# 3DTopia/3DTopia-XL

Measured on AMD Instinct MI355X. Metric: DiT denoise-steps/sec (N_prim=2048) + samples/sec @25-step DDIM, higher is better.
Workload: dtype f16

## Files before the change

3dtopia-xl_amd/_lib.py:

```python
from __future__ import annotations

import ctypes as C
import os
from typing import Optional

_HERE = os.path.dirname(os.path.abspath(__file__))
LIB_PATH = os.environ.get("PRIMX_LIB") or os.path.join(_HERE, "csrc", "libprimx_hip.so")

F32, F16, BF16 = 0, 1, 2
ACT_NONE, ACT_GELU_TANH, ACT_GELU_ERF = 0, 1, 2
HEADS_ROWS, HEADS_VT, HEADS_KROWS = 0, 1, 2
ABI_VERSION = 30

_p, _i, _l, _f, _d = C.c_void_p, C.c_int, C.c_int64, C.c_float, C.c_double



class DitBlockFold(C.Structure):
    _fields_ = [(n, _p) for n in ("w_q", "b_q", "w_cproj", "b_cproj", "w_qkv", "w_proj", "b_proj", "w_fc1", "w_fc2", "b_fc2",
                                  "Kc", "Vc", "Kb", "Vb", "uv_q", "uv_qkv", "uv_fc1",
                                  "carry_q", "carry_cproj", "carry_fc1", "carry_fc2")] + \
               [(n, _l) for n in ("carry_q_bytes", "carry_cproj_bytes", "carry_fc1_bytes", "carry_fc2_bytes")]


class F32outProblem(C.Structure):
    _fields_ = [("A", _p), ("W", _p), ("bias", _p), ("out", _p), ("N", _i), ("first_wg", _i)]


class DitForwardFold(C.Structure):
    _fields_ = [(n, _i) for n in ("dtype", "Be", "N", "D", "H", "dh", "hidden", "depth", "L", "nq_pad", "nkv_pad_c", "nkv_pad_b",
                                  "b_from", "step", "n_steps")] + \
               [("ln_eps", _f), ("scale", _f)] + \
               [(n, _p) for n in ("h", "xn", "att", "hid", "Qc", "Qs", "Ks", "Vs", "mod", "center0", "center1", "part")] + \
               [(n, _p) for n in ("kv_A", "kv_W", "kv_bias")] + [(n, _i) for n in ("kv_rows", "kv_rows_per_batch", "kv_K")]


SIGNATURES = {
    "primx_dit_blocks_fold": [C.POINTER(DitForwardFold), C.POINTER(DitBlockFold), _p],
    "primx_abi_version": [],
    "primx_last_error": [],
    "primx_last_gemm_kernel": [],
    "primx_padded_head_dim": [_i],
    "primx_layernorm_modulate": [_p, _p, _p, _l, _p, _i, _i, _i, _i, _f, _p, _l, _p, _l, _p],
    "primx_timestep_embedding": [_p, _p, _p, _i, _i, _p],
    "primx_compute_raydirs": [_p, _p, _p, _p, _p, _f, _p, _p, _p, _i, _i, _i, _p],
    "primx_raymarch": [_p, _p, _p, _f, _p, _p, _p, _p, _p, _i, _i, _i, _i, _i, _i, _i, _f, _f, _p],
    "primx_primsdf_query": [_p, _p, _p, _p, _p, _i, _i, _i, _i, _i, _p],
    "primx_vit_tokens": [_p, _p, _p, _p, _p, _i, _i, _i, _i, _p],
    "primx_point_features": [_p, _l, _p, _p, _l, _i, _i, _p],
    "primx_prefetch": [_p, _l, _p],
    "primx_silu_cast": [_p, _p, _i, _l, _p],
    "primx_cast16": [_p, _p, _i, _l, _p],
    "primx_linear_f32": [_p, _p, _p, _p, _p, _i, _i, _i, _i, _p],
    "primx_linear": [_p, _p, _p, _p, _i, _i, _i, _i, _i, _f, _p, _l, _p],
    "primx_linear_gate_residual": [_p, _p, _p, _p, _l, _p, _i, _i, _i, _i, _i, _p, _l, _p],
    "primx_linear_gate_residual_ln": [_p, _p, _p, _p, _l, _p, _i, _i, _i, _i, _p, _p, _l, _p, _f, _p, _l, _i, _p, _l, _p],
    "primx_ln_sync_timeouts": [],
    "primx_linear_f32out": [_p, _p, _p, _p, _i, _i, _i, _i, _i, _p],
    "primx_row_stats": [_p, _i, _i, _f, _p, _p],
    "primx_linear_gate_residual_fold": [_p, _p, _p, _p, _l, _p, _i, _i, _i, _i, _p, _l, _p, _p, _p, _i, _p, _l, _p],
    "primx_linear_heads_fold": [_p, _p, _i, _i, _i, _i, _i, _i, _i, C.POINTER(_i), C.POINTER(_p), _i, _f, _p, _p, _p, _p, _p, _f,
                                _i, _p, _l, _p],
    "primx_linear_heads_fold_pair": [_p, _p, _i, _i, _i, _i, _i, _i, _i, C.POINTER(_i), C.POINTER(_p), _i, _f, _p, _p, _p, _p, _p, _f,
                                     _p, _p, _p, _i, _i, _i, _i, _i, _i, _i, C.POINTER(_i), C.POINTER(_p), _i, _f, _i, _p],
    "primx_linear_f32out_group": [_p, _i, _i, _i, _i, _i, _i, _p],
    "primx_linear_fold": [_p, _p, _p, _i, _i, _i, _i, _p, _p, _p, _p, _p, _f, _i, _p, _l, _p],
    "primx_linear_heads": [_p, _p, _p, _i, _i, _i, _i, _i, _i, _i, C.POINTER(_i), C.POINTER(_p), _i, _i, _i, _f, _i, _p, _l, _p],
    "primx_attention": [_p, _p, _p, _p, _i, _i, _i, _i, _i, _i, _i, _f, _i, _p],
    "primx_attention_bcast": [_p, _p, _p, _p, _i, _i, _i, _i, _i, _i, _i, _f, _p, _p, _i, _i, _i, _p],
    "primx_pack_heads": [_p, _l, _l, _l, _p, _i, _i, _i, _i, _i, _i, _i, _p],
    "primx_cfg_combine": [_p, _p, _i, _l, _f, _p],
    "primx_diffusion_step": [_p, _p, _i, _l, _i, _i, _p, _i, _i, _i, _i, _i, _p, _p, _p, _p],
    "primx_groupnorm_silu": [_p, _p, _p, _p, _i, _i, _i, _i, _f, _i, _i, _p],
    "primx_conv3d_k3": [_p, _p, _p, _p, _f, _p, _i, _i, _i, _i, _i, _i, _p],
    "primx_conv3d_s4_pack": [_p, _p, _i, _i, _p],
    "primx_conv3d_s4_packed": [_p, _p, _p, _p, _f, _p, _i, _i, _i, _p],
    "primx_conv3d_s8_pack": [_p, _p, _p, _i, _p],
    "primx_conv3d_s8_fused": [_p, _p, _p, _p, _p, _p, _p, _f, _p, _p, _p, _i, _i, _p],
    "primx_conv3d_s8_packed": [_p, _p, _p, _p, _f, _p, _i, _i, _p],
    "primx_convtranspose_s4_pack": [_p, _p, _i, _p],
    "primx_convtranspose_s4_packed": [_p, _p, _p, _p, _p, _i, _i, _p],
    "primx_conv3d_s8c32_pack": [_p, _p, _i, _i, _i, _p],
    "primx_conv3d_s8c32_packed": [_p, _p, _p, _p, _p, _f, _p, _f, _p, _i, _i, _i, _p],
    "primx_linear_residual": [_p, _p, _p, _p, _f, _p, _i, _i, _i, _i, _p],
    "primx_conv_in": [_p, _f, _f, _p, _p, _p, _i, _i, _i, _i, _p],
    "primx_convtranspose_k2s2": [_p, _p, _p, _p, _i, _i, _i, _i, _i, _p],
    "primx_vae_output": [_p, _p, _i, _i, _i, _i, _f, _i, _p],
    "primx_latent_denorm": [_p, _p, _p, _f, _p, _p, _l, _i, _i, _p],
    "primx_gemm_f32": [_p, _p, _p, _p, _i, _i, _i, _i, _f, _p, _l, _i, _p],
    "primx_attention_f32": [_p, _p, _p, _p, _i, _i, _i, _i, _i, C.POINTER(_l), C.POINTER(_l), C.POINTER(_l), _f, _p],
    "primx_layernorm_modulate_f32": [_p, _p, _p, _l, _p, _i, _i, _i, _f, _p],
    "primx_silu_f32": [_p, _p, _l, _p],
    "primx_mcubes_workspace": [_i, _i, _i, C.POINTER(_l)],
    "primx_mcubes_count": [_p, _i, _i, _i, _f, _p, _l, _p, _p],
    "primx_mcubes_emit": [_p, _i, _i, _i, _f, _p, _l, _l, _l, _p, _p, _p, _p],
    "primx_noise_filter": [_p, _i, _p, _p],
    "primx_texbake_labels": [_p, _p, _p, _i, _i, _p, _p],
    "primx_texbake_components_workspace": [_i, _i, C.POINTER(_l)],
    "primx_texbake_components": [_p, _i, _i, _p, _l, _p, C.POINTER(_l), _p],
    "primx_texbake_raster_workspace": [_i, _i, C.POINTER(_l)],
    "primx_texbake_raster": [_p, _p, _i, _i, _i, _i, _p, _p, _p, _l, _p, _p],
    "primx_texbake_compact": [_p, _i, _i, _p, _l, _p, _p, _i, _p, _p, _i, _i, _l, _p, _p, _p],
    "primx_texbake_fill_workspace": [_i, _i, C.POINTER(_l)],
    "primx_texbake_fill": [_p, _p, _l, _p, _i, _i, _i, _i, _p, _l, _p, _p, _p],
    "primx_meshclean_workspace": [_i, _i, C.POINTER(_l)],
    "primx_meshclean_merge": [_p, _p, _i, _i, _d, _p, _l, _p, C.POINTER(_l), C.POINTER(_f), _p],
    "primx_meshclean_faces": [_p, _p, _p, _i, _i, _p, _l, _p, C.POINTER(_l), _p],
    "primx_meshclean_components": [_p, _p, _p, _p, _i, _i, _i, _i, _i, _d, _i, _p, _l, _p, _p, _p, C.POINTER(_l), _p],
    "primx_meshclean_edges": [_p, _p, _i, _i, _p, _l, _p, _l, _p, C.POINTER(_l), _p],
    "primx_meshclean_fans": [_p, _p, _i, _i, _i, _p, _l, _p, _p, C.POINTER(_l), _p],
    "primx_meshdecim_workspace": [_i, _i, C.POINTER(_l)],
    "primx_meshdecim_edges": [_p, _p, _p, _i, _i, _i, _p, _p, _p, _p, _p],
    "primx_meshdecim_quadrics": [_p, _p, _p, _p, _p, _p, _p, _i, _i, _i, _p, _p, _p],
    "primx_meshdecim_costs": [_p, _p, _p, _p, _p, _i, _i, _i, _p, _p, _p, _p, _p],
    "primx_meshdecim_select": [_p, _p, _p, _p, _p, _p, _p, _p, _p, _p, _p, _i, _i, _i, _i, _p, _p, _p, _p],
    "primx_meshdecim_collapse": [_p, _p, _p, _p, _p, _p, _p, _p, _p, _p, _p, _i, _i, _i, _i, _i, _p, _l, _p, C.POINTER(_l), _p],
    "primx_meshdecim_finish": [_p, _p, _i, _i, _p, _l, _p, _p, _p, C.POINTER(_l), _p],
    "primx_meshdecim_normals": [_p, _p, _p, _p, _i, _i, _p, _l, _p, _p],
}
_RESTYPES = {"primx_last_error": C.c_char_p, "primx_last_gemm_kernel": C.c_char_p}
_FOLD_ENTRY_POINTS: set = {"primx_linear_f32out", "primx_row_stats", "primx_linear_gate_residual_fold", "primx_linear_heads_fold",
                           "primx_linear_fold"}
_MESH_ENTRY_POINTS: set = {"primx_mcubes_workspace", "primx_mcubes_count", "primx_mcubes_emit", "primx_noise_filter"}
_TEXBAKE_ENTRY_POINTS: set = {"primx_texbake_labels", "primx_texbake_components_workspace", "primx_texbake_components",
                              "primx_texbake_raster_workspace", "primx_texbake_raster", "primx_texbake_compact",
                              "primx_texbake_fill_workspace", "primx_texbake_fill"}
_MESHCLEAN_ENTRY_POINTS: set = {"primx_meshclean_workspace", "primx_meshclean_merge", "primx_meshclean_faces",
                                "primx_meshclean_components", "primx_meshclean_edges", "primx_meshclean_fans"}
_MESHDECIM_ENTRY_POINTS: set = {"primx_meshdecim_workspace", "primx_meshdecim_edges", "primx_meshdecim_quadrics",
                                "primx_meshdecim_costs", "primx_meshdecim_select", "primx_meshdecim_collapse",
                                "primx_meshdecim_finish", "primx_meshdecim_normals"}
_AB_ABI_VERSIONS: tuple = (21, 22, 23, 24, 25, 26, 27, 28, 29)
_fold_available: dict = {}
_blocks_call: dict = {}
_kv_ride: dict = {}
_f32out_group: dict = {}

_lib: Optional[C.CDLL] = None


class PrimxError(RuntimeError):
    """A C-ABI entry point returned a non-zero status."""


def load(path: Optional[str] = None) -> C.CDLL:
    global _lib
    if _lib is not None and path is None:
        return _lib
    path = path or LIB_PATH
    if not os.path.exists(path):
        raise RuntimeError(
            f"{path} not found: the HIP library is not built. Run `python __graft_entry__.py` "
            "(build()) first - there is no PyTorch/CPU fallback for this path."
        )
    if path == LIB_PATH and not os.environ.get("PRIMX_LIB") and not os.environ.get("PRIMX_SKIP_FRESH_CHECK"):
        import importlib.util
        spec = importlib.util.spec_from_file_location("primx_build", os.path.join(_HERE, "csrc", "build.py"))
        mod = importlib.util.module_from_spec(spec)
        spec.loader.exec_module(mod)
        if not mod.check_fresh():
            raise RuntimeError(f"{path} does not match the sources in {os.path.dirname(path)} (build_manifest.json): "
                               "run `python __graft_entry__.py` (build()) to rebuild it")
    try:
        import torch
    except Exception:
        pass
    lib = C.CDLL(path)
    ab = bool(os.environ.get("PRIMX_LIB"))
    lib.primx_abi_version.restype = C.c_int
    got = lib.primx_abi_version()
    if got != ABI_VERSION and not (ab and got in _AB_ABI_VERSIONS):
        raise RuntimeError(f"libprimx_hip.so ABI {got} != expected {ABI_VERSION}; rebuild it")
    for name, argtypes in SIGNATURES.items():
        if got < 23 and name in _FOLD_ENTRY_POINTS:
            continue
        if got < 24 and name == "primx_dit_blocks_fold":
            continue
        if got < 25 and name == "primx_linear_heads_fold_pair":
            continue
        if got < 26 and name == "primx_linear_f32out_group":
            continue
        if got < 27 and name in _MESH_ENTRY_POINTS:
            continue
        if got < 28 and name in _TEXBAKE_ENTRY_POINTS:
            continue
        if got < 29 and name in _MESHCLEAN_ENTRY_POINTS:
            continue
        if got < 30 and name in _MESHDECIM_ENTRY_POINTS:
            continue
        fn = getattr(lib, name)
        fn.argtypes = argtypes
        fn.restype = _RESTYPES.get(name, C.c_int)
    _fold_available[path] = got >= 23
    _blocks_call[path] = got >= 24
    _kv_ride[path] = got >= 25
    _f32out_group[path] = got >= 26
    if path == LIB_PATH:
        _lib = lib
    return lib


def fold_available() -> bool:
    load()
    return _fold_available.get(LIB_PATH, False)


def blocks_call_available() -> bool:
    load()
    return _blocks_call.get(LIB_PATH, False)


def kv_ride_available() -> bool:
    load()
    return _kv_ride.get(LIB_PATH, False)


def f32out_group_available() -> bool:
    load()
    return _f32out_group.get(LIB_PATH, False)


def check(status: int, name: str) -> None:
    if status != 0:
        msg = load().primx_last_error()
        raise PrimxError(f"{name} failed ({status}): {msg.decode() if msg else '?'}")
```

3dtopia-xl_amd/csrc/build.py:

```python
from __future__ import annotations

import hashlib
import json
import os
import subprocess
import sys
from concurrent.futures import ThreadPoolExecutor

HERE = os.path.dirname(os.path.abspath(__file__))
SOURCES = ["rowops.hip", "gemm.hip", "attention.hip", "vae.hip", "primsdf.hip", "raymarch.hip", "fp32.hip", "conv3.hip", "conv3s8.hip", "conv3s8c32.hip", "convt.hip", "dit_host.hip", "mcubes.hip", "texbake.hip", "meshclean.hip", "meshdecim.hip"]
HEADERS = ["common.h", "ln_row.h", "gemm288q_body.inc", "mc_tables.h", "block_scan.h", os.path.join("..", "..", "include", "primx_hip.h")]
LIB = os.path.join(HERE, "libprimx_hip.so")
MANIFEST = os.path.join(HERE, "build_manifest.json")
FLAGS = ["--offload-arch=gfx950", "-O3", "-std=c++17", "-fPIC", "-fno-gpu-rdc", "-Wall", "-Wno-unused-function",
         "-mllvm", "-amdgpu-kernarg-preload-count=16"]
EXTRA_FLAGS: dict = {}


def _hipcc() -> str:
    for c in (os.environ.get("HIPCC"), "/opt/rocm/bin/hipcc", "hipcc"):
        if c and (os.path.isabs(c) and os.path.exists(c) or not os.path.isabs(c)):
            return c
    raise RuntimeError("hipcc not found")


def _sha(paths, extra: str = "") -> str:
    h = hashlib.sha256(extra.encode())
    for p in paths:
        with open(p, "rb") as f:
            h.update(hashlib.sha256(f.read()).digest())
    return h.hexdigest()


def source_hashes() -> dict:
    hdrs = [os.path.join(HERE, h) for h in HEADERS]
    out = {}
    for src in SOURCES:
        out[src.replace(".hip", ".o")] = _sha([os.path.join(HERE, src)] + hdrs, " ".join(FLAGS + EXTRA_FLAGS.get(src, [])))
    out["lib"] = hashlib.sha256("".join(out[k] for k in sorted(out)).encode()).hexdigest()
    return out


def _manifest() -> dict:
    try:
        with open(MANIFEST) as f:
            return json.load(f)
    except (OSError, ValueError):
        return {}


def check_fresh() -> bool:
    if not os.path.exists(LIB):
        return False
    return _manifest().get("lib") == source_hashes()["lib"]


def build(force: bool = False, verbose: bool = True) -> str:
    want, have = source_hashes(), _manifest()
    objs, jobs, names = [], [], []
    for src in SOURCES:
        name = src.replace(".hip", ".o")
        o = os.path.join(HERE, name)
        objs.append(o)
        if force or not os.path.exists(o) or have.get(name) != want[name]:
            jobs.append((name, [_hipcc(), *FLAGS, *EXTRA_FLAGS.get(src, []), "-c", os.path.join(HERE, src), "-o", o]))
            names.append(name)

    def run(cmd):
        if verbose:
            print(" ".join(cmd), flush=True)
        subprocess.run(cmd, check=True, cwd=HERE)

    done = dict(have)
    if jobs:
        done.pop("lib", None)
        with ThreadPoolExecutor(max_workers=4) as ex:
            list(ex.map(lambda j: run(j[1]), jobs))
        for name in names:
            done[name] = want[name]
    if force or jobs or not os.path.exists(LIB) or have.get("lib") != want["lib"]:
        run([_hipcc(), "--offload-arch=gfx950", "-shared", "-fPIC", "-o", LIB, *objs])
        done["lib"] = want["lib"]
        with open(MANIFEST, "w") as f:
            json.dump({k: done[k] for k in sorted(done) if k in want}, f, indent=1)
    return LIB


if __name__ == "__main__":
    print(build(force="--force" in sys.argv))
```

3dtopia-xl_amd/csrc/dit_host.hip:

```cpp
#include <stdint.h>

#include "common.h"

#define PRIMX_FAIL(...)               \
    do {                              \
        primx_set_error(__VA_ARGS__); \
        return PRIMX_EINVAL;          \
    } while (0)

extern "C" int primx_dit_blocks_fold(const PrimxDitForwardFold* f, const PrimxDitBlockFold* blocks, void* stream) {
    if (!f || !blocks) PRIMX_FAIL("primx_dit_blocks_fold: null descriptor");
    if (f->dtype != PRIMX_F16 && f->dtype != PRIMX_BF16) PRIMX_FAIL("primx_dit_blocks_fold: dtype must be PRIMX_F16 or PRIMX_BF16");
    if (f->depth <= 0 || f->Be <= 0 || f->N <= 0 || f->D <= 0 || f->H <= 0 || f->dh * f->H != f->D || f->hidden <= 0)
        PRIMX_FAIL("primx_dit_blocks_fold: bad shape (depth %d, Be %d, N %d, D %d, H %d, dh %d, hidden %d)", f->depth, f->Be, f->N, f->D,
                   f->H, f->dh, f->hidden);
    if (f->step < 0 || f->step >= f->n_steps) PRIMX_FAIL("primx_dit_blocks_fold: step %d outside the u / v tables (%d rows)", f->step, f->n_steps);
    if (f->b_from < 0 || f->b_from > f->Be) PRIMX_FAIL("primx_dit_blocks_fold: b_from %d outside [0, %d]", f->b_from, f->Be);
    if (!f->h || !f->xn || !f->att || !f->hid || !f->Qc || !f->Qs || !f->Ks || !f->Vs || !f->mod || !f->center0 || !f->center1 || !f->part)
        PRIMX_FAIL("primx_dit_blocks_fold: null workspace");
    const int dt = f->dtype, Be = f->Be, N = f->N, D = f->D, H = f->H, dh = f->dh, T = Be * N;
    const char* mod = static_cast<const char*>(f->mod);
    auto ch = [&](int i, int j) -> const void* { return mod + ((int64_t)(i * 9 + j) * D) * 2; };
    float* center[2] = {f->center0, f->center1};
    int side = 0;
    const int kq[1] = {PRIMX_HEADS_ROWS}, kqkv[3] = {PRIMX_HEADS_ROWS, PRIMX_HEADS_KROWS, PRIMX_HEADS_VT};
    void* const dq[1] = {f->Qc};
    void* const dqkv[3] = {f->Qs, f->Ks, f->Vs};
    auto uv = [&](const float* base, int n_site, const float*& u, const float*& v) {
        u = base + (int64_t)f->step * n_site;
        v = base + ((int64_t)f->n_steps + f->step) * n_site;
    };
    int rc;
#define PRIMX_DIT_CALL(x)          \
    do {                           \
        rc = (x);                  \
        if (rc != PRIMX_OK) return rc; \
    } while (0)
    const int kkv[2] = {PRIMX_HEADS_KROWS, PRIMX_HEADS_VT};
    if (f->kv_A) {
        if (!f->kv_W || f->kv_rows <= 0 || f->kv_rows_per_batch <= 0 || f->kv_rows % f->kv_rows_per_batch || f->kv_K <= 0)
            PRIMX_FAIL("primx_dit_blocks_fold: bad K / V projection (rows %d, rows per batch entry %d, K %d)", f->kv_rows, f->kv_rows_per_batch, f->kv_K);
        for (int i = 0; i < f->depth; ++i)
            if (!blocks[i].Kc || !blocks[i].Vc) PRIMX_FAIL("primx_dit_blocks_fold: block %d: null K / V destination", i);
    }
    const char* const kvW = static_cast<const char*>(f->kv_W);
    const char* const kvB = static_cast<const char*>(f->kv_bias);
#define PRIMX_DIT_KV(i)                                                                                                                      \
    f->kv_A, kvW + (int64_t)(i) * 2 * D * f->kv_K * 2, kvB ? kvB + (int64_t)(i) * 2 * D * 2 : nullptr, f->kv_rows, 2 * D, f->kv_K,         \
        f->kv_rows_per_batch, H, dh, 2, kkv, kvdst, f->nkv_pad_c, 1.0f
    if (f->kv_A) {
        void* const kvdst[2] = {const_cast<void*>(blocks[0].Kc), const_cast<void*>(blocks[0].Vc)};
        PRIMX_DIT_CALL(primx_linear_heads_fold_pair(nullptr, nullptr, 0, 0, 0, 0, 0, 0, 0, nullptr, nullptr, 0, 0.f, nullptr, nullptr, nullptr, nullptr,
                                                    nullptr, 0.f, PRIMX_DIT_KV(0), dt, stream));
    }
    for (int i = 0; i < f->depth; ++i) {
        const PrimxDitBlockFold& b = blocks[i];
        if (!b.w_q || !b.w_cproj || !b.w_qkv || !b.w_proj || !b.w_fc1 || !b.w_fc2 || !b.uv_qkv || !b.uv_fc1 || (i > 0 && !b.uv_q))
            PRIMX_FAIL("primx_dit_blocks_fold: block %d: null weight or table", i);
        const float *u, *v;
        if (i == 0) {
            PRIMX_DIT_CALL(primx_layernorm_modulate(f->h, ch(0, 0), ch(0, 1), 0, f->xn, dt, T, N, D, f->ln_eps, nullptr, 0, nullptr, 0, stream));
            PRIMX_DIT_CALL(primx_row_stats(f->h, T, D, f->ln_eps, center[0], stream));
            side = 0;
        }
        if (b.uv_q) {
            uv(b.uv_q, D, u, v);
            PRIMX_DIT_CALL(primx_linear_heads_fold(f->xn, b.w_q, T, D, D, N, H, dh, 1, kq, dq, f->nq_pad, f->scale, f->part, u, v, center[side],
                                                   center[side ^ 1], f->ln_eps, dt, b.carry_q, b.carry_q_bytes, stream));
            side ^= 1;
        } else {
            PRIMX_DIT_CALL(primx_linear_heads(f->xn, b.w_q, b.b_q, T, D, D, N, H, dh, 1, kq, dq, 1, 0, f->nq_pad, f->scale, dt, b.carry_q,
                                              b.carry_q_bytes, stream));
        }
        if (f->b_from < Be) {
            if (!b.Kb || !b.Vb || (f->b_from > 0 && (!b.Kc || !b.Vc))) PRIMX_FAIL("primx_dit_blocks_fold: block %d: null cross-attention operand", i);
            PRIMX_DIT_CALL(primx_attention_bcast(f->Qc, f->b_from > 0 ? b.Kc : nullptr, f->b_from > 0 ? b.Vc : nullptr, f->att, Be, H, N, f->nq_pad,
                                                 f->L, f->b_from > 0 ? f->nkv_pad_c : f->nkv_pad_b, dh, f->scale, b.Kb, b.Vb, f->b_from,
                                                 f->nkv_pad_b, dt, stream));
        } else {
            if (!b.Kc || !b.Vc) PRIMX_FAIL("primx_dit_blocks_fold: block %d: null cross-attention operand", i);
            PRIMX_DIT_CALL(primx_attention(f->Qc, b.Kc, b.Vc, f->att, Be, H, N, f->nq_pad, f->L, f->nkv_pad_c, dh, f->scale, dt, stream));
        }
        PRIMX_DIT_CALL(primx_linear_gate_residual_fold(f->att, b.w_cproj, b.b_cproj, ch(i, 2), 0, f->h, T, D, D, N, ch(i, 4), 0, center[side], f->xn,
                                                       f->part, dt, b.carry_cproj, b.carry_cproj_bytes, stream));
        uv(b.uv_qkv, 3 * D, u, v);
        if (f->kv_A && i + 1 < f->depth) {
            void* const kvdst[2] = {const_cast<void*>(blocks[i + 1].Kc), const_cast<void*>(blocks[i + 1].Vc)};
            PRIMX_DIT_CALL(primx_linear_heads_fold_pair(f->xn, b.w_qkv, T, 3 * D, D, N, H, dh, 3, kqkv, dqkv, f->nq_pad, 1.0f, f->part, u, v,
                                                        center[side], center[side ^ 1], f->ln_eps, PRIMX_DIT_KV(i + 1), dt, stream));
        } else {
            PRIMX_DIT_CALL(primx_linear_heads_fold(f->xn, b.w_qkv, T, 3 * D, D, N, H, dh, 3, kqkv, dqkv, f->nq_pad, 1.0f, f->part, u, v, center[side],
                                                   center[side ^ 1], f->ln_eps, dt, nullptr, 0, stream));
        }
        side ^= 1;
        PRIMX_DIT_CALL(primx_attention(f->Qs, f->Ks, f->Vs, f->att, Be, H, N, f->nq_pad, N, f->nq_pad, dh, f->scale, dt, stream));
        PRIMX_DIT_CALL(primx_linear_gate_residual_fold(f->att, b.w_proj, b.b_proj, ch(i, 5), 0, f->h, T, D, D, N, ch(i, 7), 0, center[side], f->xn,
                                                       f->part, dt, nullptr, 0, stream));
        uv(b.uv_fc1, f->hidden, u, v);
        PRIMX_DIT_CALL(primx_linear_fold(f->xn, b.w_fc1, f->hid, T, f->hidden, D, PRIMX_ACT_GELU_TANH, f->part, u, v, center[side], center[side ^ 1],
                                         f->ln_eps, dt, b.carry_fc1, b.carry_fc1_bytes, stream));
        side ^= 1;
        if (i + 1 < f->depth) {
            PRIMX_DIT_CALL(primx_linear_gate_residual_fold(f->hid, b.w_fc2, b.b_fc2, ch(i, 8), 0, f->h, T, D, f->hidden, N, ch(i + 1, 1), 0,
                                                           center[side], f->xn, f->part, dt, b.carry_fc2, b.carry_fc2_bytes, stream));
        } else {
            PRIMX_DIT_CALL(primx_linear_gate_residual_ln(f->hid, b.w_fc2, b.b_fc2, ch(i, 8), 0, f->h, T, D, f->hidden, N, ch(f->depth, 0),
                                                         ch(f->depth, 1), 0, f->xn, f->ln_eps, nullptr, 0, dt, nullptr, 0, stream));
        }
    }
#undef PRIMX_DIT_KV
#undef PRIMX_DIT_CALL
    return PRIMX_OK;
}
```

3dtopia-xl_amd/csrc/ln_row.h:

```cpp
#pragma once
#include "common.h"

__device__ __forceinline__ float half_wave_sum(float v) {
#pragma unroll
    for (int off = 16; off > 0; off >>= 1) v += __shfl_xor(v, off);
    return v;
}

template <int DT, int NCH4>
__device__ __forceinline__ void ln_row32(const float* __restrict__ xr, const typename T16<DT>::S* __restrict__ sh,
                                         const typename T16<DT>::S* __restrict__ sc, typename T16<DT>::S* __restrict__ orow,
                                         int l32, float eps) {
    using S = typename T16<DT>::S;
    using V4 = typename T16<DT>::V4;
    constexpr int D = NCH4 * 128;
    xr += l32 * 4;
    f32x4 v[NCH4];
    float s = 0.f;
#pragma unroll
    for (int c = 0; c < NCH4; ++c) {
        v[c] = *reinterpret_cast<const f32x4*>(xr + c * 128);
        s += (v[c][0] + v[c][1]) + (v[c][2] + v[c][3]);
    }
    const float mean = half_wave_sum(s) * (1.0f / D);
    float q = 0.f;
#pragma unroll
    for (int c = 0; c < NCH4; ++c)
#pragma unroll
        for (int j = 0; j < 4; ++j) {
            const float a = v[c][j] - mean;
            q += a * a;
        }
    const float rstd = 1.0f / sqrtf(half_wave_sum(q) * (1.0f / D) + eps);
    sh += l32 * 4;
    sc += l32 * 4;
    orow += l32 * 4;
#pragma unroll
    for (int c = 0; c < NCH4; ++c) {
        const V4 s4 = *reinterpret_cast<const V4*>(sc + c * 128);
        const V4 h4 = *reinterpret_cast<const V4*>(sh + c * 128);
        V4 o;
#pragma unroll
        for (int j = 0; j < 4; ++j) {
            const float m1 = rnd16<DT>(1.0f + (float)s4[j]);
            o[j] = (S)((v[c][j] - mean) * rstd * m1 + (float)h4[j]);
        }
        *reinterpret_cast<V4*>(orow + c * 128) = o;
    }
}
```

3dtopia-xl_amd/dit.py:

```python
from __future__ import annotations

import math
import os
from typing import Dict, Optional

import torch
from torch import nn

import ctypes as C

from . import _lib, ops
from ._lib import ACT_GELU_TANH, HEADS_KROWS, HEADS_ROWS, HEADS_VT
from .attention import MemEffAttention, MemEffCrossAttention, _c16


def modulate(x, shift, scale):
    return x * (1 + scale.unsqueeze(1)) + shift.unsqueeze(1)


class TimestepEmbedder(nn.Module):

    def __init__(self, hidden_size: int, frequency_embedding_size: int = 256):
        super().__init__()
        self.mlp = nn.Sequential(
            nn.Linear(frequency_embedding_size, hidden_size, bias=True),
            nn.SiLU(),
            nn.Linear(hidden_size, hidden_size, bias=True),
        )
        self.frequency_embedding_size = frequency_embedding_size

    @staticmethod
    def timestep_embedding(t: torch.Tensor, dim: int, max_period: float = 10000) -> torch.Tensor:
        if dim % 2:
            raise NotImplementedError("odd embedding sizes are not used on this path")
        return ops.timestep_embedding(t, dim, float(max_period))

    def forward(self, t: torch.Tensor) -> torch.Tensor:
        f = self.timestep_embedding(t, self.frequency_embedding_size)
        h = ops.linear_f32(f, self.mlp[0].weight.detach(), self.mlp[0].bias.detach(), act_out=1)
        return ops.linear_f32(h, self.mlp[2].weight.detach(), self.mlp[2].bias.detach())


class Mlp(nn.Module):

    def __init__(self, in_features: int, hidden_features: Optional[int] = None, out_features: Optional[int] = None,
                 act_layer=None, norm_layer=None, bias: bool = True, drop: float = 0.0, use_conv: bool = False):
        super().__init__()
        if use_conv or norm_layer is not None or drop:
            raise NotImplementedError("only the Linear / no-norm / no-dropout Mlp of the DiT block is supported")
        out_features = out_features or in_features
        hidden_features = hidden_features or in_features
        self.fc1 = nn.Linear(in_features, hidden_features, bias=bias)
        self.fc2 = nn.Linear(hidden_features, out_features, bias=bias)


class DiTBlock(nn.Module):

    def __init__(self, hidden_size, cross_attn_cond_dim, num_heads, mlp_ratio=4.0, proj_bias=False,
                 gradient_checkpointing=False, **block_kwargs):
        super().__init__()
        self.gradient_checkpointing = gradient_checkpointing
        self.crossattn = MemEffCrossAttention(dim=hidden_size, dim_q=hidden_size, dim_k=cross_attn_cond_dim,
                                              dim_v=cross_attn_cond_dim, num_heads=num_heads, qkv_bias=True,
                                              proj_bias=proj_bias, **block_kwargs)
        self.attn = MemEffAttention(dim=hidden_size, num_heads=num_heads, qkv_bias=True, proj_bias=proj_bias,
                                    **block_kwargs)
        self.mlp = Mlp(in_features=hidden_size, hidden_features=int(hidden_size * mlp_ratio))
        self.adaLN_modulation = nn.Sequential(nn.SiLU(), nn.Linear(hidden_size, 9 * hidden_size, bias=True))


class FinalLayer(nn.Module):

    def __init__(self, hidden_size, seq_length, out_channels):
        super().__init__()
        self.linear = nn.Linear(hidden_size, out_channels, bias=True)
        self.adaLN_modulation = nn.Sequential(nn.SiLU(), nn.Linear(hidden_size, 2 * hidden_size, bias=True))


class DiT(nn.Module):

    LN_EPS = 1e-6

    def __init__(self, seq_length=2, in_channels=4, condition_channels=512, hidden_size=1152, depth=28,
                 num_heads=16, mlp_ratio=4.0, cond_drop_prob=0.0, attn_proj_bias=False, learn_sigma=True,
                 gradient_checkpointing=False):
        super().__init__()
        self.gradient_checkpointing = gradient_checkpointing
        self.learn_sigma = learn_sigma
        self.in_channels = in_channels
        self.out_channels = in_channels * 2 if learn_sigma else in_channels
        self.seq_length = seq_length
        self.num_heads = num_heads
        self.hidden_size = hidden_size
        self.depth = depth
        self.condition_channels = condition_channels
        self.cond_drop_prob = cond_drop_prob
        if self.cond_drop_prob > 0:
            self.null_cond_embedding = nn.Parameter(torch.randn(condition_channels))
        self.x_embedder = nn.Linear(in_channels, hidden_size)
        self.t_embedder = TimestepEmbedder(hidden_size)
        self.blocks = nn.ModuleList([
            DiTBlock(hidden_size, condition_channels, num_heads, mlp_ratio=mlp_ratio, proj_bias=attn_proj_bias,
                     gradient_checkpointing=gradient_checkpointing) for _ in range(depth)
        ])
        self.final_layer = FinalLayer(hidden_size, seq_length, self.out_channels)
        self.initialize_weights()
        self._pack: Dict = {}
        self._heads_ws: Dict = {}
        self._heads_owner: Dict = {}
        self._heads_lru: list = []
        self._heads_group = None
        self._cond: Optional[Dict] = None
        self._packed_only = False
        self.reuse_cond_kv = False
        self.collapse_null_cross_attention = False
        self.cfg_streams = os.environ.get("PRIMX_CFG_STREAMS") == "1"
        self.dedup_null_kv = os.environ.get("PRIMX_NULL_KV_DEDUP", "1") != "0"
        self.weight_prefetch = int(os.environ.get("PRIMX_WPREFETCH", "2"))
        self.fuse_ln = os.environ.get("PRIMX_DIT_FUSE_LN", "1") != "0"
        self.ln_in_kernel = os.environ.get("PRIMX_DIT_LN_TAIL", "0") == "1"
        self._ln_sync: Dict = {}
        self.fold_ln = os.environ.get("PRIMX_DIT_FOLD", "1") != "0"
        self._fold_ws: Dict = {}
        self.fold_max_steps = int(os.environ.get("PRIMX_DIT_FOLD_MAX_STEPS", "128"))
        self.blocks_call = os.environ.get("PRIMX_DIT_BLOCKS_CALL", "1") != "0"
        self.kv_ride = os.environ.get("PRIMX_DIT_KV_RIDE", "1") != "0"
        self._fold_fp16_used = False
        self.block_probe: Optional[list] = None
        self._side: Dict = {}
        self._t_plan: Optional[Dict] = None

    def initialize_weights(self):
        for m in self.modules():
            if isinstance(m, nn.Linear):
                nn.init.xavier_uniform_(m.weight)
                if m.bias is not None:
                    nn.init.zeros_(m.bias)
        nn.init.normal_(self.t_embedder.mlp[0].weight, std=0.02)
        nn.init.normal_(self.t_embedder.mlp[2].weight, std=0.02)
        for blk in self.blocks:
            nn.init.zeros_(blk.adaLN_modulation[-1].weight)
            nn.init.zeros_(blk.adaLN_modulation[-1].bias)
        nn.init.zeros_(self.final_layer.adaLN_modulation[-1].weight)
        nn.init.zeros_(self.final_layer.adaLN_modulation[-1].bias)
        nn.init.zeros_(self.final_layer.linear.weight)
        nn.init.zeros_(self.final_layer.linear.bias)

    def repack(self) -> None:
        self._t_plan = None
        self._pack = {}
        self._heads_ws, self._heads_owner, self._heads_lru, self._heads_group = {}, {}, [], None
        self._cond = None
        self._packed_only = False

    def _apply(self, fn, *a, **k):
        self.__dict__["_pack"] = {}
        self.__dict__["_heads_ws"] = {}
        self.__dict__["_heads_owner"] = {}
        self.__dict__["_heads_lru"] = []
        self.__dict__["_heads_group"] = None
        self.__dict__["_cond"] = None
        self.__dict__["_t_plan"] = None
        return super()._apply(fn, *a, **k)

    def load_state_dict(self, *a, **k):
        self.repack()
        return super().load_state_dict(*a, **k)

    _PACK_ALIGN = 128

    def _pack_layout(self):
        D, Dc, depth = self.hidden_size, self.condition_channels, self.depth
        Hm = self.blocks[0].mlp.fc1.out_features if depth else 0
        proj_bias = depth > 0 and self.blocks[0].attn.proj.bias is not None
        items = []
        for i in range(depth):
            items += [("w_q", i, (D, D)), ("b_q", i, (D,)), ("w_cproj", i, (D, D)), ("b_cproj", i, (D,) if proj_bias else None),
                      ("w_qkv", i, (3 * D, D)), ("b_qkv", i, (3 * D,)), ("w_proj", i, (D, D)),
                      ("b_proj", i, (D,) if proj_bias else None), ("w_fc1", i, (Hm, D)), ("b_fc1", i, (Hm,)),
                      ("w_fc2", i, (D, Hm)), ("b_fc2", i, (D,))]
        items += [("w_kv_all", None, (depth * 2 * D, Dc) if depth else None), ("b_kv_all", None, (depth * 2 * D,) if depth else None),
                  ("w_ada", None, (depth * 9 * D + 2 * D, D)), ("b_ada", None, (depth * 9 * D + 2 * D,)),
                  ("w_final", None, (self.out_channels, D)), ("b_final", None, (self.out_channels,))]
        return items

    def packed_alloc(self, dtype: torch.dtype, device=None) -> Dict:
        device = self.x_embedder.weight.device if device is None else torch.device(device)
        layout = self._pack_layout()
        al = self._PACK_ALIGN
        total = sum(ops.round_up(math.prod(shp), al) for _, _, shp in layout if shp is not None)
        flat = torch.zeros(total, dtype=dtype, device=device)
        pk: Dict = {"blocks": [dict() for _ in range(self.depth)], "_flat": flat}
        off = 0
        for name, blk, shp in layout:
            view = None
            if shp is not None:
                n = math.prod(shp)
                view = flat[off:off + n].view(shp)
                off += ops.round_up(n, al)
            (pk if blk is None else pk["blocks"][blk])[name] = view
        self._pack = {(dtype, device): pk}
        self._cond = None
        return pk

    def packed(self, dtype: torch.dtype) -> Dict:
        dev = self.x_embedder.weight.device
        key = (dtype, dev)
        if key in self._pack:
            return self._pack[key]
        if self._packed_only:
            raise RuntimeError(f"this module holds only packed 16-bit weights (broadcast_packed_ / pack_from_state_dict / "
                               f"load_packed), and not for ({dtype}, {dev}): the fp32 parameters were never loaded")
        pk = self.packed_alloc(dtype, dev)
        self._fill_pack(pk, lambda prm: prm)
        return pk

    def _fill_pack(self, pk: Dict, src) -> None:
        D = self.hidden_size
        with torch.no_grad():
            for i, blk in enumerate(self.blocks):
                ca, sa, mlp, w = blk.crossattn, blk.attn, blk.mlp, pk["blocks"][i]
                for name, lin in (("q", ca.to_q), ("cproj", ca.proj), ("qkv", sa.qkv), ("proj", sa.proj), ("fc1", mlp.fc1),
                                  ("fc2", mlp.fc2)):
                    w["w_" + name].copy_(src(lin.weight))
                    if w["b_" + name] is not None:
                        w["b_" + name].copy_(src(lin.bias))
                pk["w_kv_all"][i * 2 * D:i * 2 * D + D].copy_(src(ca.to_k.weight))
                pk["w_kv_all"][i * 2 * D + D:(i + 1) * 2 * D].copy_(src(ca.to_v.weight))
                pk["b_kv_all"][i * 2 * D:i * 2 * D + D].copy_(src(ca.to_k.bias))
                pk["b_kv_all"][i * 2 * D + D:(i + 1) * 2 * D].copy_(src(ca.to_v.bias))
                pk["w_ada"][i * 9 * D:(i + 1) * 9 * D].copy_(src(blk.adaLN_modulation[1].weight))
                pk["b_ada"][i * 9 * D:(i + 1) * 9 * D].copy_(src(blk.adaLN_modulation[1].bias))
            base = self.depth * 9 * D
            pk["w_ada"][base:].copy_(src(self.final_layer.adaLN_modulation[1].weight))
            pk["b_ada"][base:].copy_(src(self.final_layer.adaLN_modulation[1].bias))
            pk["w_final"].copy_(src(self.final_layer.linear.weight))
            pk["b_final"].copy_(src(self.final_layer.linear.bias))

    def pack_from_state_dict(self, state_dict: Dict, dtype: torch.dtype, device=None) -> Dict:
        names = {id(prm): n for n, prm in self.named_parameters()}
        missing = [n for n in names.values() if n not in state_dict]
        known = set(names.values()) | {n for n, _ in self.named_buffers()}
        extra = [k for k in state_dict if k not in known]
        if missing or extra:
            raise RuntimeError(f"pack_from_state_dict: missing keys {missing[:4]}{'...' if len(missing) > 4 else ''}, "
                               f"unexpected keys {extra[:4]}{'...' if len(extra) > 4 else ''}")
        for prm in self.parameters():
            if tuple(state_dict[names[id(prm)]].shape) != tuple(prm.shape):
                raise RuntimeError(f"pack_from_state_dict: shape mismatch for {names[id(prm)]}: checkpoint "
                                   f"{tuple(state_dict[names[id(prm)]].shape)}, model {tuple(prm.shape)}")
        self.repack()
        pk = self.packed_alloc(dtype, device)
        self._fill_pack(pk, lambda prm: state_dict[names[id(prm)]])
        with torch.no_grad():
            for t, prm in zip(self.small_fp32_tensors(), self._small_fp32_params()):
                t.copy_(state_dict[names[id(prm)]])
        self._packed_only = True
        return pk

    PACKED_MAGIC = b"PRIMXPK1"
    PACKED_FORMAT = 2
    _PACKED_FILE_ALIGN = 4096

    def _hyper(self) -> Dict:
        proj_bias = self.depth > 0 and self.blocks[0].attn.proj.bias is not None
        return {"class": type(self).__name__, "seq_length": self.seq_length, "in_channels": self.in_channels, "condition_channels": self.condition_channels,
                "hidden_size": self.hidden_size, "depth": self.depth, "num_heads": self.num_heads,
                "mlp_hidden": self.blocks[0].mlp.fc1.out_features if self.depth else 0, "attn_proj_bias": bool(proj_bias),
                "cond_drop_prob_positive": self.cond_drop_prob > 0, "out_channels": self.out_channels}

    def save_packed(self, path: str, dtype: torch.dtype) -> int:
        import json
        pk = self.packed(dtype)
        flat = pk["_flat"].detach().cpu().contiguous()
        small = [t.detach().cpu().float().contiguous() for t in self.small_fp32_tensors()]
        al = self._PACKED_FILE_ALIGN
        head = {"format": self.PACKED_FORMAT, "dtype": str(dtype).replace("torch.", ""), "hyper": self._hyper(), "pack_align": self._PACK_ALIGN,
                "blob_elements": flat.numel(),
                "small_fp32": [list(t.shape) for t in small]}
        hj = json.dumps(head, sort_keys=True).encode()
        blob_off = ops.round_up(16 + len(hj), al)
        blob_bytes = flat.numel() * flat.element_size()
        small_off = ops.round_up(blob_off + blob_bytes, al)
        with open(path, "wb") as f:
            f.write(self.PACKED_MAGIC)
            f.write(len(hj).to_bytes(8, "little"))
            f.write(hj)
            f.write(b"\0" * (blob_off - 16 - len(hj)))
            raw = flat.view(torch.int16).numpy()
            for lo in range(0, raw.size, 1 << 25):
                f.write(raw[lo:lo + (1 << 25)].tobytes())
            f.write(b"\0" * (small_off - blob_off - blob_bytes))
            for t in small:
                f.write(t.numpy().tobytes())
            return f.tell()

    def load_packed(self, path: str, device=None) -> Dict:
        import json
        import os
        with open(path, "rb") as f:
            if f.read(8) != self.PACKED_MAGIC:
                raise RuntimeError(f"{path}: not a packed PrimX DiT file")
            hlen = int.from_bytes(f.read(8), "little")
            head = json.loads(f.read(hlen).decode())
        if head.get("format") != self.PACKED_FORMAT:
            raise RuntimeError(f"{path}: packed file format {head.get('format')} (this build reads format {self.PACKED_FORMAT}): "
                               "repack required - write it again with DiT.save_packed from the checkpoint")
        if head.get("hyper") != self._hyper() or head.get("pack_align") != self._PACK_ALIGN:
            raise RuntimeError(f"{path}: packed for a different model ({head.get('hyper')}) than this one ({self._hyper()})")
        dtype = {"float16": torch.float16, "bfloat16": torch.bfloat16}[head["dtype"]]
        self.repack()
        pk = self.packed_alloc(dtype, device)
        flat = pk["_flat"]
        if flat.numel() != head["blob_elements"]:
            raise RuntimeError(f"{path}: blob has {head['blob_elements']} elements, this model's layout {flat.numel()}")
        al = self._PACKED_FILE_ALIGN
        blob_off = ops.round_up(16 + hlen, al)
        blob_bytes = flat.numel() * flat.element_size()
        small_off = ops.round_up(blob_off + blob_bytes, al)
        mm = torch.from_file(path, shared=False, size=os.path.getsize(path), dtype=torch.uint8)
        with torch.no_grad():
            flat.view(torch.int16).copy_(mm[blob_off:blob_off + blob_bytes].view(torch.int16))
            off = small_off
            for t, shp in zip(self.small_fp32_tensors(), head["small_fp32"]):
                if list(t.shape) != shp:
                    raise RuntimeError(f"{path}: fp32 tensor of shape {shp} does not fit {list(t.shape)}")
                n = t.numel()
                t.copy_(mm[off:off + 4 * n].view(torch.float32).view(shp))
                off += 4 * n
        del mm
        self._packed_only = True
        return pk

    def _small_fp32_params(self):
        ps = [self.x_embedder.weight, self.x_embedder.bias, self.t_embedder.mlp[0].weight, self.t_embedder.mlp[0].bias,
              self.t_embedder.mlp[2].weight, self.t_embedder.mlp[2].bias]
        if self.cond_drop_prob > 0:
            ps.append(self.null_cond_embedding)
        return ps

    def small_fp32_tensors(self):
        return [t.data for t in self._small_fp32_params()]

    def _heads(self, tag: str, B: int, n: int, kind: int, dtype, device, pad_to: int) -> torch.Tensor:
        key = (tag, B, n, kind, dtype, str(device), pad_to)
        buf = self._heads_ws.get(key)
        if buf is None:
            buf = ops.alloc_heads(B, self.num_heads, n, self.hidden_size // self.num_heads, kind, dtype, device, pad_to,
                                  role=tag[0].lower())
            self._heads_ws[key] = buf
        self._heads_owner.setdefault(key, set()).add(self._heads_group)
        return buf

    _HEADS_GROUPS = 3

    def _heads_begin(self, group) -> None:
        lru = self._heads_lru
        if group in lru:
            lru.remove(group)
        lru.append(group)
        self._heads_group = group
        while len(lru) > self._HEADS_GROUPS:
            old = lru.pop(0)
            for k in [k for k, gs in self._heads_owner.items() if old in gs]:
                gs = self._heads_owner[k]
                gs.discard(old)
                if not gs:
                    self._heads_ws.pop(k, None)
                    self._heads_owner.pop(k, None)

    def _side_stream(self, dev) -> "torch.cuda.Stream":
        key = str(dev)
        if key not in self._side:
            self._side[key] = torch.cuda.Stream(device=dev)
        return self._side[key]

    def _cond_state(self, y: torch.Tensor, null_half: bool, dt) -> Dict:
        B, L, Dc = y.shape
        Be = 2 * B if null_half else B
        st = self._cond
        ver = None if y.is_inference() else y._version
        if st is not None and ver is not None:
            k = st["y"]
            if (k.data_ptr() == y.data_ptr() and k.shape == y.shape and k.stride() == y.stride() and k.dtype == y.dtype
                    and st["ver"] == ver and st["dt"] == dt and st["null_half"] == null_half):
                return st
        Lk = L
        if (ops.round_up(L, 256) - L) * 8 <= L:
            Lk = ops.round_up(L, 256)
        buf = torch.zeros(Be, Lk, Dc, dtype=dt, device=y.device)
        yf = y.float().contiguous()
        for b in range(B):
            ops.cast16(yf[b], dt, out=buf[b, :L])
        if null_half:
            null16 = ops.cast16(self.null_cond_embedding.detach().float().contiguous().to(y.device), dt)
            buf[B:, :L] = null16
        st = {"y": y, "ver": ver, "dt": dt, "null_half": null_half, "Lk": Lk, "y16": buf.view(Be * Lk, Dc),
              "kv_valid": False, "null16": None}
        if null_half and L >= 64:
            st["null16"] = null16.reshape(1, Dc).expand(ops.bcast_keys(L), Dc).contiguous()
        self._cond = st
        return st

    @ops.on_input_device
    def forward(self, x, t, y, precision_dtype=torch.float32, enable_amp=False):
        self._check_inputs(x)
        if not enable_amp or precision_dtype == torch.float32:
            return self._forward_fp32(x, t, y)
        if precision_dtype not in (torch.float16, torch.bfloat16):
            raise NotImplementedError(f"autocast dtype {precision_dtype} is not supported (fp16 / bf16 / fp32)")
        return self._forward16(x, t, y, precision_dtype, null_half=False)

    def _check_inputs(self, x):
        if self.training:
            raise NotImplementedError("the accelerated DiT is inference-only: call .eval()")
        if not x.is_cuda:
            raise RuntimeError("DiT.forward needs HIP device tensors; there is no CPU path")

    _PLAN_ROWS = 8

    def plan_timesteps(self, timesteps: torch.Tensor) -> None:
        if timesteps.dim() != 1 or timesteps.dtype != torch.int64 or not timesteps.is_cuda:
            raise RuntimeError("plan_timesteps: expected a 1-D int64 HIP device tensor")
        self._t_plan = {"t": timesteps.contiguous(), "mod": {}, "row": None}

    def select_planned_timestep(self, row: Optional[int]) -> None:
        if self._t_plan is not None:
            if row is not None and not (0 <= row < self._t_plan["t"].numel()):
                raise IndexError(f"planned timestep {row} out of range")
            self._t_plan["row"] = row

    def clear_timestep_plan(self) -> None:
        self._t_plan = None
        self._fold_fp16_used = False

    def _modulation_table(self, plan: Dict, dt: torch.dtype, pk: Dict) -> torch.Tensor:
        key = (dt, pk["w_ada"].data_ptr())
        tab = plan["mod"].get(key)
        if tab is None:
            ts = plan["t"]
            n, R = ts.numel(), self._PLAN_ROWS
            tab = torch.empty(n, pk["w_ada"].shape[0], dtype=dt, device=ts.device)
            for lo in range(0, n, R):
                st16 = ops.silu_cast(self.t_embedder(ts[lo:lo + R]), dt)
                ops.linear(st16, pk["w_ada"], pk["b_ada"], out=tab[lo:lo + R])
            plan["mod"] = {key: tab}
        return tab

    def _fold_ok(self, T: int, N: int) -> bool:
        return bool(self.fold_ln) and self.depth > 0 and ops.fold_shapes_ok(T, N, self.hidden_size, self.num_heads)

    def _fold_tables(self, plan: Dict, dt: torch.dtype, pk: Dict) -> Dict:
        key = (dt, pk["w_ada"].data_ptr())
        ft = plan.get("fold")
        if ft is not None and ft["key"] == key:
            return ft
        tab = self._modulation_table(plan, dt, pk)
        n, D = tab.shape[0], self.hidden_size
        A = self._fold_rows(tab, self.depth, D)
        sites, uv = [], []
        total = sum(2 * n * w["w_" + name].shape[0] for i, w in enumerate(pk["blocks"]) for s, name in enumerate(("q", "qkv", "fc1"))
                    if not (i == 0 and s == 0))
        flat, off = torch.empty(total, dtype=torch.float32, device=tab.device), 0
        for i, w in enumerate(pk["blocks"]):
            row = []
            for s, name in enumerate(("q", "qkv", "fc1")):
                if i == 0 and s == 0:
                    row.append(None)
                    continue
                Ns = w["w_" + name].shape[0]
                out = flat[off:off + 2 * n * Ns].view(2, n, Ns)
                off += 2 * n * Ns
                sites.append((A[i, s].view(2 * n, D), w["w_" + name], w["b_" + name], out.view(2 * n, Ns)))
                row.append(out)
            uv.append(row)
        if not ops.linear_f32out_group(sites, bias_from_row=n):
            for a_s, w_s, b_s, o_s in sites:
                ops.linear_f32out(a_s, w_s, b_s, o_s, bias_from_row=n)
        ft = plan["fold"] = {"key": key, "uv": uv}
        return ft

    def fold_overflowed(self, sample: torch.Tensor) -> bool:
        used, self._fold_fp16_used = self._fold_fp16_used, False
        return bool(used) and not bool(torch.isfinite(sample).all())

    @staticmethod
    def _fold_rows(tab: torch.Tensor, depth: int, D: int) -> torch.Tensor:
        n = tab.shape[0]
        v = tab[:, :depth * 9 * D].view(n, depth, 3, 3, D)
        A = torch.empty(depth, 3, 2, n, D, dtype=tab.dtype, device=tab.device)
        A[:, :, 0] = (1 + v[:, :, :, 1]).permute(1, 2, 0, 3)
        A[:, :, 1] = v[:, :, :, 0].permute(1, 2, 0, 3)
        return A

    def _forward16(self, x, t, y, dt, null_half: bool):
        B, N, Cin = x.shape
        Be = 2 * B if null_half else B
        L, Dc = y.shape[1], y.shape[2]
        D, H = self.hidden_size, self.num_heads
        dh = D // H
        T = Be * N
        pk = self.packed(dt)
        dev = x.device
        self._heads_begin((Be, N, L, dt, str(dev)))

        xf = x.reshape(B * N, Cin).float().contiguous()
        h = torch.empty(T, D, dtype=torch.float32, device=dev)
        self._embed_tokens(xf, h[:B * N], h[B * N:] if null_half else None)
        plan = self._t_plan
        if plan is not None and plan["row"] is not None:
            mod = self._modulation_table(plan, dt, pk)[plan["row"]:plan["row"] + 1].expand(Be, -1)
        else:
            t_emb = self.t_embedder(t)
            st16 = torch.empty(Be, D, dtype=dt, device=dev)
            ops.silu_cast(t_emb, dt, out=st16[:B])
            if null_half:
                ops.silu_cast(t_emb, dt, out=st16[B:])
            mod = ops.linear(st16, pk["w_ada"], pk["b_ada"])
        cs = self._cond_state(y, null_half, dt)
        cs["group"] = self._heads_group
        Lk, y16 = cs["Lk"], cs["y16"]

        nq_pad = ops.round_up(N, ops.BQ)
        Qc = self._heads("Qc", Be, N, HEADS_ROWS, dt, dev, ops.BQ)
        kv_pad = 256 if Lk != L else ops.BKV
        dedup = bool(self.dedup_null_kv) and null_half and cs["null16"] is not None and self.depth > 0
        Bkv = B if dedup else Be
        Kc = self._heads("Kc", self.depth * Bkv, L, HEADS_KROWS, dt, dev, kv_pad)
        Vc = self._heads("Vc", self.depth * Bkv, L, HEADS_VT, dt, dev, kv_pad)
        Kc_blk = Kc.view(self.depth, Bkv, *Kc.shape[1:])
        Vc_blk = Vc.view(self.depth, Bkv, *Vc.shape[1:])
        Kn_blk = Vn_blk = None
        if dedup:
            Ln = ops.bcast_keys(L)
            Kn = self._heads("Kn", self.depth, Ln, HEADS_KROWS, dt, dev, ops.BKV)
            Vn = self._heads("Vn", self.depth, Ln, HEADS_VT, dt, dev, ops.BKV)
            Kn_blk, Vn_blk = Kn.view(self.depth, 1, *Kn.shape[1:]), Vn.view(self.depth, 1, *Vn.shape[1:])
        need_kv = bool(self.depth) and not (self.reuse_cond_kv and cs["kv_valid"] and cs.get("kv_id") == (Kc.data_ptr(), Vc.data_ptr()))

        ride_state = {"on": False}

        def kv_problem(i: int):
            wkv, bkv = pk["w_kv_all"][i * 2 * D:(i + 1) * 2 * D], pk["b_kv_all"][i * 2 * D:(i + 1) * 2 * D]
            return (y16[:Bkv * Lk], wkv, bkv, Lk, H, dh, [HEADS_KROWS, HEADS_VT], [Kc_blk[i], Vc_blk[i]], Kc.shape[2], 1.0, Bkv * L)

        def project_kv(cond_rows: bool) -> None:
            if cond_rows:
                ops.linear_heads(y16[:Bkv * Lk], pk["w_kv_all"], pk["b_kv_all"], Lk, H, dh, [HEADS_KROWS, HEADS_VT], [Kc, Vc],
                                 Kc.shape[2], n_rep=self.depth, rep_batches=Bkv, real_rows=Bkv * L)
            if dedup:
                ops.linear_heads(cs["null16"], pk["w_kv_all"], pk["b_kv_all"], Ln, H, dh, [HEADS_KROWS, HEADS_VT], [Kn, Vn],
                                 Kn.shape[2], n_rep=self.depth, rep_batches=1)
            cs["kv_valid"], cs["kv_id"] = True, (Kc.data_ptr(), Vc.data_ptr())
        Qs = self._heads("Qs", Be, N, HEADS_ROWS, dt, dev, ops.BQ)
        Ks = self._heads("Ks", Be, N, HEADS_KROWS, dt, dev, ops.BQ)
        Vs = self._heads("Vs", Be, N, HEADS_VT, dt, dev, ops.BQ)
        xn = torch.empty(T, D, dtype=dt, device=dev)
        att = torch.empty(Be, N, D, dtype=dt, device=dev)
        hid = torch.empty(T, pk["blocks"][0]["w_fc1"].shape[0], dtype=dt, device=dev) if self.depth else None
        scale = dh ** -0.5

        wpf = int(self.weight_prefetch)
        collapse = bool(self.collapse_null_cross_attention) and null_half
        blocks = pk["blocks"]
        fuse = bool(self.fuse_ln) and wpf != 1
        sync = None
        sync_w = ops.ln_sync_words(T)
        if fuse and self.ln_in_kernel:
            key = str(dev)
            sync = self._ln_sync.get(key)
            if sync is None or sync.numel() < 2 * sync_w:
                sync = self._ln_sync[key] = torch.zeros(2 * sync_w, dtype=torch.int32, device=dev)
        base = self.depth * 9 * D
        fin_mod = (mod[:, base:base + D], mod[:, base + D:base + 2 * D])
        fold_uv = fcent = fpart = None
        prow = plan["row"] if plan is not None else None
        if (prow is not None and fuse and not collapse and not (self.cfg_streams and null_half and ops.PROFILE is None)
                and plan["t"].numel() <= self.fold_max_steps and self._fold_ok(T, N)):
            fold_uv = self._fold_tables(plan, dt, pk)["uv"]
            if dt == torch.float16:
                self._fold_fp16_used = True
            wk = (str(dev), T)
            if wk not in self._fold_ws:
                self._fold_ws = {wk: ops.fold_workspace(T, D, dev)}
            fcent, fpart = self._fold_ws[wk]

        fside: Dict[int, int] = {}

        def warm(*wts):
            return wts if wpf == 1 else ()

        def carry(wt):
            return wt if wpf == 2 else None

        def block(i, w, b0, b1, hook=None):
            r0, r1 = b0 * N, b1 * N
            hh, xh, ah = h[r0:r1], xn[r0:r1], att[b0:b1]
            Th = r1 - r0
            m = mod[b0:b1, i * 9 * D:(i + 1) * 9 * D]
            ch = [m[:, j * D:(j + 1) * D] for j in range(9)]
            def ln_of(shift, scale):
                if not fuse:
                    return None
                return (shift, scale, xh, self.LN_EPS, None if sync is None else (sync[:sync_w] if b0 == 0 else sync[sync_w:]))
            folded = fold_uv is not None
            fp = fpart[r0:r1] if folded else None
            uvs = fold_uv[i] if folded else None

            def fc_in():
                return fcent[fside[b0]][r0:r1]

            def fc_flip():
                fside[b0] ^= 1
                return fcent[fside[b0]][r0:r1]

            def uv(s):
                return uvs[s][0, prow], uvs[s][1, prow]
            if not fuse or i == 0:
                ops.layernorm_modulate(hh, ch[0], ch[1], N, xh, self.LN_EPS, prefetch=warm(w["w_q"], w["w_cproj"]))
                if folded:
                    fside[b0] = 0
                    ops.row_stats(hh, self.LN_EPS, fc_in())
            bc = min(b1, B) if collapse else b1
            if bc > b0:
                if folded and i > 0:
                    ops.linear_heads_fold(xh, w["w_q"], N, H, dh, [HEADS_ROWS], [Qc[b0:bc]], nq_pad, fp, *uv(0), fc_in(), fc_flip(),
                                          self.LN_EPS, scale0=scale, carry=carry(w["w_cproj"]))
                else:
                    ops.linear_heads(xh[:(bc - b0) * N], w["w_q"], w["b_q"], N, H, dh, [HEADS_ROWS], [Qc[b0:bc]], nq_pad,
                                     scale0=scale, carry=carry(w["w_cproj"]))
                if dedup and bc > B:
                    kc = Kc_blk[i][b0:B] if b0 < B else None
                    ops.attention(Qc[b0:bc], kc, Vc_blk[i][b0:B] if b0 < B else None, N, L, dh, scale, out=ah[:bc - b0],
                                  bcast=(Kn_blk[i], Vn_blk[i]))
                else:
                    ops.attention(Qc[b0:bc], Kc_blk[i][b0:bc], Vc_blk[i][b0:bc], N, L, dh, scale, out=ah[:bc - b0])
            if bc < b1:
                nb = b1 - max(bc, b0)
                vsrc = Vn_blk[i].expand(nb, -1, -1, -1) if dedup else Vc_blk[i][max(bc, b0):b1]
                vrow = vsrc[:, :, :dh, 0].reshape(nb, 1, D)
                ah[max(bc, b0) - b0:].copy_(vrow.expand(-1, N, -1))
            if hook is not None:
                hook()
            if folded:
                ops.linear_gate_residual_fold(ah.view(Th, D), w["w_cproj"], w["b_cproj"], ch[2], hh, N, ch[4], fc_in(), xh, fp,
                                              carry=carry(w["w_proj"]))
            else:
                ops.linear_gate_residual(ah.view(Th, D), w["w_cproj"], w["b_cproj"], ch[2], hh, N, carry=carry(w["w_proj"]),
                                         ln=ln_of(ch[3], ch[4]))
            if not fuse:
                ops.layernorm_modulate(hh, ch[3], ch[4], N, xh, self.LN_EPS, prefetch=warm(w["w_proj"]))
            if folded and ride_state["on"] and i + 1 < len(blocks):
                u1, v1 = uv(1)
                ops.linear_heads_fold_pair(dict(A=xh, W=w["w_qkv"], rows_per_batch=N, heads=H, dh=dh, kinds=[HEADS_ROWS, HEADS_KROWS, HEADS_VT],
                                                dsts=[Qs[b0:b1], Ks[b0:b1], Vs[b0:b1]], n_pad=nq_pad, part=fp, u=u1, v=v1, center=fc_in(),
                                                center_out=fc_flip(), eps=self.LN_EPS), *kv_problem(i + 1))
            elif folded:
                ops.linear_heads_fold(xh, w["w_qkv"], N, H, dh, [HEADS_ROWS, HEADS_KROWS, HEADS_VT],
                                      [Qs[b0:b1], Ks[b0:b1], Vs[b0:b1]], nq_pad, fp, *uv(1), fc_in(), fc_flip(), self.LN_EPS)
            else:
                ops.linear_heads(xh, w["w_qkv"], w["b_qkv"], N, H, dh, [HEADS_ROWS, HEADS_KROWS, HEADS_VT],
                                 [Qs[b0:b1], Ks[b0:b1], Vs[b0:b1]], nq_pad)
            ops.attention(Qs[b0:b1], Ks[b0:b1], Vs[b0:b1], N, N, dh, scale, out=ah)
            if folded:
                ops.linear_gate_residual_fold(ah.view(Th, D), w["w_proj"], w["b_proj"], ch[5], hh, N, ch[7], fc_in(), xh, fp)
            else:
                ops.linear_gate_residual(ah.view(Th, D), w["w_proj"], w["b_proj"], ch[5], hh, N, ln=ln_of(ch[6], ch[7]))
            if not fuse:
                ops.layernorm_modulate(hh, ch[6], ch[7], N, xh, self.LN_EPS, prefetch=warm(w["w_fc2"]))
            if folded:
                ops.linear_fold(xh, w["w_fc1"], hid[r0:r1], fp, *uv(2), fc_in(), fc_flip(), self.LN_EPS, act=ACT_GELU_TANH,
                                carry=carry(w["w_fc2"]))
            else:
                ops.linear(xh, w["w_fc1"], w["b_fc1"], out=hid[r0:r1], act=ACT_GELU_TANH, carry=carry(w["w_fc2"]))
            last = i + 1 == len(blocks)
            nxt = (fin_mod[0][b0:b1], fin_mod[1][b0:b1]) if last else \
                (mod[b0:b1, (i + 1) * 9 * D:(i + 1) * 9 * D + D], mod[b0:b1, (i + 1) * 9 * D + D:(i + 1) * 9 * D + 2 * D])
            if folded and not last:
                ops.linear_gate_residual_fold(hid[r0:r1], w["w_fc2"], w["b_fc2"], ch[8], hh, N, nxt[1], fc_in(), xh, fp,
                                              carry=carry(blocks[i + 1]["w_q"]))
            else:
                ops.linear_gate_residual(hid[r0:r1], w["w_fc2"], w["b_fc2"], ch[8], hh, N,
                                         carry=None if last else carry(blocks[i + 1]["w_q"]), ln=ln_of(*nxt))

        two_streams = bool(self.cfg_streams and null_half and self.depth and ops.PROFILE is None)
        one_call = (not two_streams and fold_uv is not None and self.blocks_call and sync is None and ops.PROFILE is None
                    and self.block_probe is None and _lib.blocks_call_available())
        ride = (need_kv and self.kv_ride and fold_uv is not None and not two_streams and _lib.kv_ride_available()
                and ops.fold_pair_fits(T, N, D, H, Bkv * Lk, Lk, Dc))
        ride_state["on"] = ride and not one_call
        if need_kv:
            project_kv(not ride)
            if ride_state["on"]:
                ops.linear_heads_fold_pair(None, *kv_problem(0))
        if self.cfg_streams and null_half and self.depth and ops.PROFILE is None:
            main = torch.cuda.current_stream()
            side = self._side_stream(dev)
            side.wait_stream(main)
            lag = torch.cuda.Event()
            for i, w in enumerate(pk["blocks"]):
                block(i, w, 0, B, hook=(lambda: lag.record(main)) if i == 0 else None)
                with torch.cuda.stream(side):
                    if i == 0:
                        side.wait_event(lag)
                    block(i, w, B, Be)
            main.wait_stream(side)
        elif one_call:
            fd = plan["fold"]
            dkey = (Kc.data_ptr(), Vc.data_ptr(), Kn_blk[0].data_ptr() if dedup else 0, wpf, Bkv)
            if fd.get("desc_key") != dkey:
                arr = (_lib.DitBlockFold * self.depth)()
                rng = lambda t: ops._range(t) if wpf == 2 else (None, 0)
                for i, w in enumerate(blocks):
                    d = arr[i]
                    for name in ("w_q", "b_q", "w_cproj", "b_cproj", "w_qkv", "w_proj", "b_proj", "w_fc1", "w_fc2", "b_fc2"):
                        setattr(d, name, None if w[name] is None else w[name].data_ptr())
                    d.Kc, d.Vc = Kc_blk[i].data_ptr(), Vc_blk[i].data_ptr()
                    d.Kb, d.Vb = (Kn_blk[i].data_ptr(), Vn_blk[i].data_ptr()) if dedup else (None, None)
                    d.uv_q = None if fold_uv[i][0] is None else fold_uv[i][0].data_ptr()
                    d.uv_qkv, d.uv_fc1 = fold_uv[i][1].data_ptr(), fold_uv[i][2].data_ptr()
                    for cname, t in (("carry_q", w["w_cproj"]), ("carry_cproj", w["w_proj"]), ("carry_fc1", w["w_fc2"]),
                                     ("carry_fc2", blocks[i + 1]["w_q"] if i + 1 < self.depth else None)):
                        cp, cn = rng(t) if t is not None else (None, 0)
                        setattr(d, cname, cp)
                        setattr(d, cname + "_bytes", cn)
                fd["desc"], fd["desc_key"] = arr, dkey
            f = _lib.DitForwardFold(
                dtype=ops.dtype_code(dt), Be=Be, N=N, D=D, H=H, dh=dh, hidden=hid.shape[1], depth=self.depth, L=L, nq_pad=nq_pad,
                nkv_pad_c=Kc.shape[2], nkv_pad_b=Kn_blk[0].shape[2] if dedup else 0, b_from=B if dedup else Be, step=prow,
                n_steps=plan["t"].numel(), ln_eps=self.LN_EPS, scale=scale, h=h.data_ptr(), xn=xn.data_ptr(), att=att.data_ptr(),
                hid=hid.data_ptr(), Qc=Qc.data_ptr(), Qs=Qs.data_ptr(), Ks=Ks.data_ptr(), Vs=Vs.data_ptr(), mod=mod.data_ptr(),
                center0=fcent[0].data_ptr(), center1=fcent[1].data_ptr(), part=fpart.data_ptr())
            if ride:
                f.kv_A, f.kv_W, f.kv_bias = y16.data_ptr(), pk["w_kv_all"].data_ptr(), pk["b_kv_all"].data_ptr()
                f.kv_rows, f.kv_rows_per_batch, f.kv_K = Bkv * Lk, Lk, Dc
            ops._dev(h, "h", torch.float32)
            _lib.check(_lib.load().primx_dit_blocks_fold(C.byref(f), fd["desc"], ops._stream()), "primx_dit_blocks_fold")
        else:
            for i, w in enumerate(pk["blocks"]):
                block(i, w, 0, Be)
                if self.block_probe is not None:
                    rs = h.std(-1)
                    self.block_probe.append({
                        "block": i, "folded": fold_uv is not None, "dtype": str(dt).replace("torch.", ""),
                        "residual_abs_max": float(h.abs().max()), "row_std_min": float(rs.min()), "row_std_median": float(rs.median()),
                        "row_std_max": float(rs.max()), "row_mean_abs_max": float(h.mean(-1).abs().max()),
                        "next_operand_abs_max": float(xn.float().abs().max()), "next_operand_finite": bool(torch.isfinite(xn.float()).all())})

        if not (fuse and self.depth):
            ops.layernorm_modulate(h, fin_mod[0], fin_mod[1], N, xn, self.LN_EPS)
        out = ops.linear(xn, pk["w_final"], pk["b_final"])
        return out.view(Be, N, self.out_channels)

    def _forward_fp32(self, x, t, y):
        if self._packed_only:
            raise RuntimeError("this module holds only packed 16-bit weights (sharding.broadcast_packed_ / pack_from_state_dict "
                               "/ load_packed): the fp32 route needs the fp32 parameters - use broadcast_module_ / "
                               "load_state_dict")
        Be, N, Cin = x.shape
        L, Dc = y.shape[1], y.shape[2]
        D, H = self.hidden_size, self.num_heads
        dh = D // H
        T = Be * N
        dev = x.device
        f = lambda p: p.detach()
        h = torch.empty(T, D, dtype=torch.float32, device=dev)
        self._embed_tokens(x.reshape(T, Cin).float().contiguous(), h)
        st = ops.silu_f32(self.t_embedder(t))
        y2 = y.float().contiguous().view(Be * L, Dc)
        scale = dh ** -0.5
        xn = torch.empty(T, D, dtype=torch.float32, device=dev)
        for blk in self.blocks:
            ada = blk.adaLN_modulation[1]
            mod = ops.gemm_f32(st, f(ada.weight), f(ada.bias))
            ch = [mod[:, j * D:(j + 1) * D] for j in range(9)]
            ca, sa, mlp = blk.crossattn, blk.attn, blk.mlp
            bias = lambda lin: None if lin.bias is None else f(lin.bias)
            ops.layernorm_modulate_f32(h, ch[0], ch[1], N, self.LN_EPS, out=xn)
            q = ops.gemm_f32(xn, f(ca.to_q.weight), bias(ca.to_q), out_scale=scale)
            k = ops.gemm_f32(y2, f(ca.to_k.weight), bias(ca.to_k))
            v = ops.gemm_f32(y2, f(ca.to_v.weight), bias(ca.to_v))
            o = ops.attention_f32(q.view(Be, N, H, dh), k.view(Be, L, H, dh), v.view(Be, L, H, dh), scale)
            ops.gemm_f32(o.view(T, D), f(ca.proj.weight), bias(ca.proj), out=h, gate=ch[2], rows_per_batch=N)
            ops.layernorm_modulate_f32(h, ch[3], ch[4], N, self.LN_EPS, out=xn)
            qkv = ops.gemm_f32(xn, f(sa.qkv.weight), bias(sa.qkv)).view(Be, N, 3, H, dh)
            o = ops.attention_f32(qkv[:, :, 0], qkv[:, :, 1], qkv[:, :, 2], scale)
            ops.gemm_f32(o.view(T, D), f(sa.proj.weight), bias(sa.proj), out=h, gate=ch[5], rows_per_batch=N)
            ops.layernorm_modulate_f32(h, ch[6], ch[7], N, self.LN_EPS, out=xn)
            hid = ops.gemm_f32(xn, f(mlp.fc1.weight), f(mlp.fc1.bias), act=ACT_GELU_TANH)
            ops.gemm_f32(hid, f(mlp.fc2.weight), f(mlp.fc2.bias), out=h, gate=ch[8], rows_per_batch=N)
        fl = self.final_layer
        mod = ops.gemm_f32(st, f(fl.adaLN_modulation[1].weight), f(fl.adaLN_modulation[1].bias))
        ops.layernorm_modulate_f32(h, mod[:, :D], mod[:, D:2 * D], N, self.LN_EPS, out=xn)
        out = ops.gemm_f32(xn, f(fl.linear.weight), f(fl.linear.bias))
        return out.view(Be, N, self.out_channels)

    def _embed_tokens(self, xf: torch.Tensor, out: torch.Tensor, out2: Optional[torch.Tensor] = None) -> torch.Tensor:
        if out2 is not None and xf.shape[0] <= 8:
            ops.linear_f32(xf, self.x_embedder.weight.detach(), self.x_embedder.bias.detach(), out=out)
            out2.copy_(out)
            return out
        return ops.linear_f32(xf, self.x_embedder.weight.detach(), self.x_embedder.bias.detach(), out=out, out2=out2)

    @ops.on_input_device
    def forward_with_cfg(self, x, t, y, cfg_scale=0.0, precision_dtype=torch.float32, enable_amp=False):
        self._check_inputs(x)
        if enable_amp and precision_dtype in (torch.float16, torch.bfloat16):
            model_out = self._forward16(x, t, y, precision_dtype, null_half=True)
        else:
            y_null = self.null_cond_embedding.detach().to(y.dtype).expand_as(y)
            model_out = self.forward(torch.cat([x, x], dim=0), torch.cat([t, t], dim=0), torch.cat([y, y_null], dim=0),
                                     precision_dtype, enable_amp)
        return ops.cfg_combine(model_out.contiguous(), float(cfg_scale))


class PointEmbed(nn.Module):

    def __init__(self, hidden_dim=48, dim=128):
        super().__init__()
        assert hidden_dim % 6 == 0
        self.embedding_dim = hidden_dim
        n = hidden_dim // 6
        e = torch.pow(2, torch.arange(n)).float() * math.pi
        z = torch.zeros(n)
        self.register_buffer("basis", torch.stack([torch.cat([e, z, z]), torch.cat([z, e, z]), torch.cat([z, z, e])]))
        self.mlp = nn.Linear(hidden_dim + 3, dim)


class DiTAdditivePosEmb(DiT):

    def __init__(self, seq_length=2, in_channels=4, condition_channels=512, hidden_size=1152, depth=28, num_heads=16,
                 mlp_ratio=4.0, attn_proj_bias=False, learn_sigma=True, gradient_checkpointing=False):
        super().__init__(seq_length=seq_length, in_channels=in_channels, condition_channels=condition_channels,
                         hidden_size=hidden_size, depth=depth, num_heads=num_heads, mlp_ratio=mlp_ratio,
                         cond_drop_prob=0.0, attn_proj_bias=attn_proj_bias, learn_sigma=learn_sigma,
                         gradient_checkpointing=gradient_checkpointing)
        self.point_emb = PointEmbed(hidden_dim=48, dim=hidden_size)

    def _embed_tokens(self, xf: torch.Tensor, out: torch.Tensor, out2: Optional[torch.Tensor] = None) -> torch.Tensor:
        pe = self.point_emb
        n = pe.embedding_dim // 6
        feat = ops.point_features(xf, pe.basis[0, :n].contiguous())
        w = pe.mlp.weight.detach()
        w = torch.nn.functional.pad(w, (0, feat.shape[1] - w.shape[1]))
        out.copy_(ops.linear_f32(xf, self.x_embedder.weight.detach(), self.x_embedder.bias.detach()) +
                  ops.linear_f32(feat, w.contiguous(), pe.mlp.bias.detach()))
        if out2 is not None:
            out2.copy_(out)
        return out

    def _small_fp32_params(self):
        return super()._small_fp32_params() + [self.point_emb.mlp.weight, self.point_emb.mlp.bias]

    def forward_with_cfg(self, *args, **kwargs):
        raise AttributeError("the reference's DiTAdditivePosEmb defines no forward_with_cfg (dit_crossattn.py:215-301)")
```

3dtopia-xl_amd/ops.py:

```python
from __future__ import annotations

import ctypes as C
import os
from typing import Optional, Sequence, Tuple

import torch

from . import _lib
from ._lib import ACT_GELU_TANH, ACT_NONE, BF16, F16, F32, HEADS_KROWS, HEADS_ROWS, HEADS_VT, check

_DT = {torch.float16: F16, torch.bfloat16: BF16, torch.float32: F32}
BQ, BKV = 128, 64


def dtype_code(dt: torch.dtype) -> int:
    try:
        return _DT[dt]
    except KeyError:
        raise TypeError(f"unsupported dtype {dt}") from None


_launch_dev: Optional[int] = None


def _dev(t: torch.Tensor, name: str, dtype: Optional[torch.dtype] = None) -> int:
    global _launch_dev
    if not t.is_cuda:
        raise RuntimeError(f"{name} must live on a HIP device (got {t.device}); there is no CPU path")
    _launch_dev = t.device.index
    if not t.is_contiguous():
        raise RuntimeError(f"{name} must be contiguous")
    if dtype is not None and t.dtype != dtype:
        raise TypeError(f"{name} must be {dtype}, got {t.dtype}")
    return t.data_ptr()


def _stream() -> int:
    cur = torch.cuda.current_device()
    if _launch_dev is not None and _launch_dev != cur:
        raise RuntimeError(f"operands live on cuda:{_launch_dev} but the current device is cuda:{cur}: call "
                           "torch.cuda.set_device(...) or wrap the call in `with torch.cuda.device(t.device)`")
    return torch.cuda.current_stream().cuda_stream


def device_of(t: torch.Tensor):
    if not t.is_cuda:
        raise RuntimeError(f"expected a HIP device tensor, got {t.device}; there is no CPU path")
    return torch.cuda.device(t.device)


def on_input_device(fn):
    import functools

    @functools.wraps(fn)
    def wrapped(*args, **kwargs):
        for a in list(args) + list(kwargs.values()):
            if isinstance(a, torch.Tensor):
                if a.is_cuda and a.device.index != torch.cuda.current_device():
                    with torch.cuda.device(a.device):
                        return fn(*args, **kwargs)
                break
        return fn(*args, **kwargs)
    return wrapped


PROFILE = None


def _timed(tag: str, flops: float, fn):
    if PROFILE is None:
        return fn()
    s, e = torch.cuda.Event(enable_timing=True), torch.cuda.Event(enable_timing=True)
    s.record()
    r = fn()
    e.record()
    if tag.startswith("None "):
        lib = _lib.load()
        name = lib.primx_last_gemm_kernel().decode() if hasattr(lib, "primx_last_gemm_kernel") else "gemm(unreported)"
        tag = name + tag[4:]
    PROFILE.append((tag, flops, s, e))
    return r


def padded_head_dim(dh: int) -> int:
    return (dh + 15) // 16 * 16


def round_up(n: int, m: int) -> int:
    return (n + m - 1) // m * m


def _range(t: Optional[torch.Tensor]) -> Tuple[Optional[int], int]:
    if t is None or not t.is_cuda or not t.is_contiguous() or t.numel() == 0:
        return None, 0
    return t.data_ptr(), t.numel() * t.element_size()


def _check_modulation(shift: torch.Tensor, scale: torch.Tensor, out: torch.Tensor) -> None:
    if shift.stride(-1) != 1 or scale.stride(-1) != 1 or shift.stride(0) != scale.stride(0):
        raise RuntimeError("shift/scale must be last-dim contiguous with equal row strides")
    if not (shift.is_cuda and scale.is_cuda and shift.dtype == out.dtype == scale.dtype):
        raise TypeError("shift/scale/out dtype or device mismatch")


def layernorm_modulate(x: torch.Tensor, shift: torch.Tensor, scale: torch.Tensor, rows_per_batch: int,
                       out: torch.Tensor, eps: float = 1e-6, prefetch: Sequence[torch.Tensor] = ()) -> torch.Tensor:
    rows, D = x.shape
    _check_modulation(shift, scale, out)
    if len(prefetch) > 2:
        raise RuntimeError("layernorm_modulate carries at most two prefetch ranges")
    (p0, n0), (p1, n1) = (_range(prefetch[0]) if len(prefetch) > 0 else (None, 0)), (_range(prefetch[1]) if len(prefetch) > 1 else (None, 0))
    check(_lib.load().primx_layernorm_modulate(
        _dev(x, "x", torch.float32), shift.data_ptr(), scale.data_ptr(), shift.stride(0), _dev(out, "out"),
        dtype_code(out.dtype), rows, rows_per_batch, D, eps, p0, n0, p1, n1, _stream()), "primx_layernorm_modulate")
    return out


_FREQS = {}


def _freq_table(dim: int, max_period: float, device) -> torch.Tensor:
    key = (dim, float(max_period), str(device))
    tab = _FREQS.get(key)
    if tab is None:
        import math
        half = dim // 2
        tab = torch.exp(-math.log(max_period) * torch.arange(start=0, end=half, dtype=torch.float32) / half).to(device)
        _FREQS[key] = tab
    return tab


def timestep_embedding(t: torch.Tensor, dim: int, max_period: float = 10000.0) -> torch.Tensor:
    t = t.to(torch.int64).contiguous()
    out = torch.empty(t.shape[0], dim, dtype=torch.float32, device=t.device)
    check(_lib.load().primx_timestep_embedding(_dev(t, "t"), _freq_table(dim, max_period, t.device).data_ptr(),
                                               out.data_ptr(), t.shape[0], dim, _stream()),
          "primx_timestep_embedding")
    return out


def point_features(x: torch.Tensor, freqs: torch.Tensor) -> torch.Tensor:
    T, F = x.shape[0], freqs.shape[0]
    if x.dim() != 2 or x.shape[1] < 4 or x.stride(1) != 1 or x.stride(0) < x.shape[1] or x.dtype != torch.float32 or not x.is_cuda:
        raise RuntimeError("point_features: x must be fp32 [T, C >= 4] on a HIP device with contiguous channels (any row stride >= C)")
    out = torch.zeros(T, round_up(6 * F + 3, 4), dtype=torch.float32, device=x.device)
    check(_lib.load().primx_point_features(x.data_ptr(), x.stride(0), _dev(freqs, "freqs", torch.float32),
                                           out.data_ptr(), out.stride(0), T, F, _stream()), "primx_point_features")
    return out


def silu_cast(x: torch.Tensor, dtype: torch.dtype, out: Optional[torch.Tensor] = None) -> torch.Tensor:
    if out is None:
        out = torch.empty(x.shape, dtype=dtype, device=x.device)
    elif out.dtype != dtype or out.numel() != x.numel() or not out.is_contiguous():
        raise RuntimeError("silu_cast: out must be a contiguous tensor of the target dtype with x.numel() elements")
    check(_lib.load().primx_silu_cast(_dev(x, "x", torch.float32), out.data_ptr(), dtype_code(dtype), x.numel(),
                                      _stream()), "primx_silu_cast")
    return out


def cast16(x: torch.Tensor, dtype: torch.dtype, out: Optional[torch.Tensor] = None) -> torch.Tensor:
    if out is None:
        out = torch.empty(x.shape, dtype=dtype, device=x.device)
    elif out.dtype != dtype or out.numel() != x.numel() or not out.is_contiguous():
        raise RuntimeError("cast16: out must be a contiguous tensor of the target dtype with x.numel() elements")
    check(_lib.load().primx_cast16(_dev(x, "x", torch.float32), out.data_ptr(), dtype_code(dtype), x.numel(),
                                   _stream()), "primx_cast16")
    return out


def linear_f32(x: torch.Tensor, W: torch.Tensor, b: Optional[torch.Tensor], act_out: int = 0,
               out: Optional[torch.Tensor] = None, out2: Optional[torch.Tensor] = None) -> torch.Tensor:
    M, K = x.shape
    N = W.shape[0]
    if out is None:
        out = torch.empty(M, N, dtype=torch.float32, device=x.device)
    for o in (out, out2):
        if o is not None and (tuple(o.shape) != (M, N) or o.dtype != torch.float32 or not o.is_contiguous()):
            raise RuntimeError("linear_f32: out / out2 must be contiguous fp32 [M, N] tensors")
    check(_lib.load().primx_linear_f32(_dev(x, "x", torch.float32), _dev(W, "W", torch.float32),
                                       _dev(b, "b", torch.float32) if b is not None else None, out.data_ptr(),
                                       _dev(out2, "out2") if out2 is not None else None, M, N, K, act_out, _stream()), "primx_linear_f32")
    return out


def prefetch(t: torch.Tensor, stream: "torch.cuda.Stream") -> None:
    check(_lib.load().primx_prefetch(_dev(t, "t"), t.numel() * t.element_size(), stream.cuda_stream), "primx_prefetch")


def linear(A: torch.Tensor, W: torch.Tensor, bias: Optional[torch.Tensor], out: Optional[torch.Tensor] = None,
           act: int = ACT_NONE, out_scale: float = 1.0, carry: Optional[torch.Tensor] = None) -> torch.Tensor:
    M, K = A.shape
    N = W.shape[0]
    if W.shape[1] != K or W.dtype != A.dtype:
        raise RuntimeError("linear: operand mismatch")
    if out is None:
        out = torch.empty(M, N, dtype=A.dtype, device=A.device)
    cp, cn = _range(carry)
    _timed(f"None {M}x{N}x{K}", 2.0 * M * N * K, lambda: check(_lib.load().primx_linear(
        _dev(A, "A"), _dev(W, "W"), _dev(bias, "bias", A.dtype) if bias is not None else None,
        _dev(out, "out", A.dtype), M, N, K, dtype_code(A.dtype), act, out_scale, cp, cn, _stream()), "primx_linear"))
    return out


def ln_sync_words(rows: int) -> int:
    return 2 * ((rows + 127) // 128)


def ln_sync_timeouts() -> int:
    return int(_lib.load().primx_ln_sync_timeouts())


def linear_gate_residual(A: torch.Tensor, W: torch.Tensor, bias: Optional[torch.Tensor], gate: torch.Tensor,
                         x: torch.Tensor, rows_per_batch: int, carry: Optional[torch.Tensor] = None,
                         ln: Optional[tuple] = None) -> torch.Tensor:
    M, K = A.shape
    N = W.shape[0]
    if gate.stride(-1) != 1 or gate.dtype != A.dtype or not gate.is_cuda:
        raise RuntimeError("gate must be a last-dim-contiguous 16-bit device view")
    cp, cn = _range(carry)
    if ln is None:
        _timed(f"None {M}x{N}x{K}", 2.0 * M * N * K, lambda: check(_lib.load().primx_linear_gate_residual(
            _dev(A, "A"), _dev(W, "W", A.dtype), _dev(bias, "bias", A.dtype) if bias is not None else None,
            gate.data_ptr(), gate.stride(0), _dev(x, "x", torch.float32), M, N, K, rows_per_batch,
            dtype_code(A.dtype), cp, cn, _stream()), "primx_linear_gate_residual"))
        return x
    shift, scale, out, eps, sync = ln
    _check_modulation(shift, scale, out)
    if PROFILE is not None and sync is None:
        linear_gate_residual(A, W, bias, gate, x, rows_per_batch, carry=carry)
        layernorm_modulate(x, shift, scale, rows_per_batch, out, eps)
        return x
    if out.dtype != A.dtype or tuple(out.shape) != (M, N):
        raise RuntimeError("linear_gate_residual: the LayerNorm output must be a 16-bit [M, N] tensor of A's dtype")
    if sync is not None and (sync.dtype != torch.int32 or not sync.is_cuda or sync.numel() < ln_sync_words(M)):
        raise RuntimeError("linear_gate_residual: sync must be an int32 device tensor of ln_sync_words(M) words")
    _timed(f"None {M}x{N}x{K}", 2.0 * M * N * K, lambda: check(_lib.load().primx_linear_gate_residual_ln(
        _dev(A, "A"), _dev(W, "W", A.dtype), _dev(bias, "bias", A.dtype) if bias is not None else None,
        gate.data_ptr(), gate.stride(0), _dev(x, "x", torch.float32), M, N, K, rows_per_batch,
        shift.data_ptr(), scale.data_ptr(), shift.stride(0), _dev(out, "ln_out"), eps,
        _dev(sync, "sync") if sync is not None else None, sync.numel() if sync is not None else 0,
        dtype_code(A.dtype), cp, cn, _stream()), "primx_linear_gate_residual_ln"))
    return x


def linear_heads(A: torch.Tensor, W: torch.Tensor, bias: Optional[torch.Tensor], rows_per_batch: int, heads: int,
                 dh: int, kinds: Sequence[int], dsts: Sequence[torch.Tensor], n_pad: int,
                 scale0: float = 1.0, n_rep: int = 1, rep_batches: int = 0, real_rows: Optional[int] = None,
                 carry: Optional[torch.Tensor] = None) -> None:
    M, K = A.shape
    N = W.shape[0]
    n_seg = len(kinds)
    kind_arr = (C.c_int * n_seg)(*kinds)
    dst_arr = (C.c_void_p * n_seg)(*[_dev(d, "dst", A.dtype) for d in dsts])
    cp, cn = _range(carry)
    _timed(f"None {M}x{N}x{K}", 2.0 * (real_rows if real_rows is not None else M) * N * K, lambda: check(_lib.load().primx_linear_heads(
        _dev(A, "A"), _dev(W, "W", A.dtype), _dev(bias, "bias", A.dtype) if bias is not None else None, M, N, K,
        rows_per_batch, heads, dh, n_seg, kind_arr, dst_arr, n_rep, rep_batches, n_pad, scale0, dtype_code(A.dtype),
        cp, cn, _stream()),
        "primx_linear_heads"))


FOLD_TILE = 144
FOLD_MAX_PARTS = 8


def fold_supported(D: int, heads: int) -> bool:
    dh = D // max(heads, 1)
    return D % FOLD_TILE == 0 and D // FOLD_TILE <= FOLD_MAX_PARTS and D % 64 == 0 and dh >= 48 and dh % 4 == 0


def fold_shapes_ok(T: int, rows_per_batch: int, D: int, heads: int) -> bool:
    if not fold_supported(D, heads) or rows_per_batch < 128 or not _lib.fold_available():
        return False
    if os.environ.get("PRIMX_GEMM_NOBIG") == "1" or os.environ.get("PRIMX_GEMM_LOADER") == "0":
        return False
    big_min = int(os.environ.get("PRIMX_GEMM_BIGHEADS_MIN", "160"))
    dh = D // heads
    return (big_min > 0 and D % 288 == 0 and 288 % dh == 0 and dh % 8 == 0 and dh >= 32 and rows_per_batch % 256 == 0
            and (T // 256) * (3 * D // 288) >= big_min)


def fold_workspace(rows: int, D: int, device) -> Tuple[torch.Tensor, torch.Tensor]:
    return (torch.empty(2, rows, 2, dtype=torch.float32, device=device),
            torch.empty(rows, D // FOLD_TILE, 2, dtype=torch.float32, device=device))


def row_stats(x: torch.Tensor, eps: float, out: torch.Tensor) -> torch.Tensor:
    rows, D = x.shape
    if tuple(out.shape) != (rows, 2):
        raise RuntimeError("row_stats: out must be [rows, 2] fp32")
    check(_lib.load().primx_row_stats(_dev(x, "x", torch.float32), rows, D, eps, _dev(out, "stats", torch.float32), _stream()),
          "primx_row_stats")
    return out


def linear_f32out(A: torch.Tensor, W: torch.Tensor, bias: Optional[torch.Tensor], out: torch.Tensor, bias_from_row: int) -> torch.Tensor:
    M, K = A.shape
    N = W.shape[0]
    if tuple(out.shape) != (M, N) or W.shape[1] != K:
        raise RuntimeError("linear_f32out: shape mismatch")
    _timed(f"None {M}x{N}x{K}", 2.0 * M * N * K, lambda: check(_lib.load().primx_linear_f32out(
        _dev(A, "A"), _dev(W, "W", A.dtype), _dev(bias, "bias", A.dtype) if bias is not None else None,
        _dev(out, "out", torch.float32), M, N, K, bias_from_row, dtype_code(A.dtype), _stream()), "primx_linear_f32out"))
    return out


def linear_f32out_group(problems: Sequence[Tuple[torch.Tensor, torch.Tensor, Optional[torch.Tensor], torch.Tensor]], bias_from_row: int) -> bool:
    if not problems or not _lib.f32out_group_available() or os.environ.get("PRIMX_UV_GROUP") == "0":
        return False
    M, K = problems[0][0].shape
    dt = problems[0][0].dtype
    dev = problems[0][0].device
    rows, first = [], 0
    flops = 0.0
    for A, W, b, out in problems:
        N = W.shape[0]
        if (tuple(A.shape) != (M, K) or A.dtype != dt or W.shape[1] != K or tuple(out.shape) != (M, N) or N % 32 or K % 32
                or not (A.is_contiguous() and W.is_contiguous() and out.is_contiguous())
                or (A.data_ptr() | W.data_ptr() | out.data_ptr()) % 16
                or any(t.device != dev for t in (A, W, out) + ((b,) if b is not None else ()))):
            return False
        rows.append([_dev(A, "A"), _dev(W, "W", dt), _dev(b, "bias", dt) if b is not None else 0, _dev(out, "out", torch.float32),
                     N | (first << 32)])
        first += (N + 127) // 128
        flops += 2.0 * M * N * K
    table = torch.tensor(rows, dtype=torch.int64).to(dev, non_blocking=False)
    _timed(f"None {len(problems)} problems x {M} rows, K = {K}", flops, lambda: check(_lib.load().primx_linear_f32out_group(
        table.data_ptr(), len(problems), first, M, K, bias_from_row, dtype_code(dt), _stream()), "primx_linear_f32out_group"))
    return True


def _fold_args(part: torch.Tensor, u: torch.Tensor, v: torch.Tensor, center: torch.Tensor, center_out: torch.Tensor, M: int, N: int,
               K: int):
    if K % FOLD_TILE or tuple(part.shape) != (M, K // FOLD_TILE, 2) or tuple(center.shape) != (M, 2) or tuple(center_out.shape) != (M, 2):
        raise RuntimeError("fold: `part` must be [M, K / 144, 2], `center` and `center_out` [M, 2] (fp32)")
    if center.data_ptr() == center_out.data_ptr():
        raise RuntimeError("fold: a consumer writes the next (centre, scale) pairs to ANOTHER array than the one it reads")
    for t, name in ((u, "u"), (v, "v")):
        if t.dtype != torch.float32 or t.numel() != N or not t.is_contiguous() or t.data_ptr() % 16:
            raise RuntimeError(f"fold: {name} must be a contiguous, 16-byte aligned fp32 vector of N elements")
    return (_dev(part, "part", torch.float32), u.data_ptr(), v.data_ptr(), _dev(center, "center", torch.float32),
            _dev(center_out, "center_out", torch.float32))


def linear_gate_residual_fold(A: torch.Tensor, W: torch.Tensor, bias: Optional[torch.Tensor], gate: torch.Tensor, x: torch.Tensor,
                              rows_per_batch: int, next_scale: torch.Tensor, center: torch.Tensor, a16: torch.Tensor,
                              part: torch.Tensor, carry: Optional[torch.Tensor] = None) -> torch.Tensor:
    M, K = A.shape
    N = W.shape[0]
    if gate.stride(-1) != 1 or gate.dtype != A.dtype or not gate.is_cuda:
        raise RuntimeError("gate must be a last-dim-contiguous 16-bit device view")
    if next_scale.stride(-1) != 1 or next_scale.dtype != A.dtype or not next_scale.is_cuda or next_scale.shape[-1] != N:
        raise RuntimeError("next_scale must be a last-dim-contiguous 16-bit device view of N columns")
    if tuple(a16.shape) != (M, N) or a16.dtype != A.dtype or tuple(part.shape) != (M, N // FOLD_TILE, 2) or \
            tuple(center.shape) != (M, 2):
        raise RuntimeError("linear_gate_residual_fold: a16 must be [M, N] 16-bit, part [M, N / 144, 2], center [M, 2]")
    cp, cn = _range(carry)
    _timed(f"None {M}x{N}x{K}", 2.0 * M * N * K, lambda: check(_lib.load().primx_linear_gate_residual_fold(
        _dev(A, "A"), _dev(W, "W", A.dtype), _dev(bias, "bias", A.dtype) if bias is not None else None,
        gate.data_ptr(), gate.stride(0), _dev(x, "x", torch.float32), M, N, K, rows_per_batch,
        next_scale.data_ptr(), next_scale.stride(0), _dev(center, "center", torch.float32), _dev(a16, "a16"),
        _dev(part, "part", torch.float32), dtype_code(A.dtype), cp, cn, _stream()), "primx_linear_gate_residual_fold"))
    return x


def linear_heads_fold(A: torch.Tensor, W: torch.Tensor, rows_per_batch: int, heads: int, dh: int, kinds: Sequence[int],
                      dsts: Sequence[torch.Tensor], n_pad: int, part: torch.Tensor, u: torch.Tensor, v: torch.Tensor,
                      center: torch.Tensor, center_out: torch.Tensor, eps: float, scale0: float = 1.0,
                      carry: Optional[torch.Tensor] = None) -> None:
    M, K = A.shape
    N = W.shape[0]
    n_seg = len(kinds)
    kind_arr = (C.c_int * n_seg)(*kinds)
    dst_arr = (C.c_void_p * n_seg)(*[_dev(d, "dst", A.dtype) for d in dsts])
    fa = _fold_args(part, u, v, center, center_out, M, N, K)
    cp, cn = _range(carry)
    _timed(f"None {M}x{N}x{K}", 2.0 * M * N * K, lambda: check(_lib.load().primx_linear_heads_fold(
        _dev(A, "A"), _dev(W, "W", A.dtype), M, N, K, rows_per_batch, heads, dh, n_seg, kind_arr, dst_arr, n_pad, scale0,
        fa[0], fa[1], fa[2], fa[3], fa[4], eps, dtype_code(A.dtype), cp, cn, _stream()), "primx_linear_heads_fold"))


def fold_pair_fits(T: int, rows_per_batch: int, D: int, heads: int, kv_rows: int, kv_rows_per_batch: int, kv_K: int) -> bool:
    if not fold_shapes_ok(T, rows_per_batch, D, heads) or os.environ.get("PRIMX_GEMM_PROF"):
        return False
    dh = D // heads
    if (2 * D) % 288 or (heads * dh) % 288 or kv_rows_per_batch % 256 or kv_rows % kv_rows_per_batch or kv_K % 64:
        return False
    g0, g1 = (T // 256) * (3 * D // 288), (kv_rows // 256) * (2 * D // 288)
    return g0 % 8 == 0 and g0 + g1 <= 256


def linear_heads_fold_pair(fold: Optional[dict], A2: torch.Tensor, W2: torch.Tensor, bias2: Optional[torch.Tensor], rows_per_batch2: int,
                           heads2: int, dh2: int, kinds2: Sequence[int], dsts2: Sequence[torch.Tensor], n_pad2: int,
                           scale0_2: float = 1.0, real_rows2: Optional[int] = None) -> None:
    M2, K2 = A2.shape
    N2 = W2.shape[0]
    fl2 = 2.0 * (real_rows2 if real_rows2 is not None else M2) * N2 * K2
    k2 = (C.c_int * len(kinds2))(*kinds2)
    d2 = (C.c_void_p * len(kinds2))(*[_dev(d, "dst", A2.dtype) for d in dsts2])
    tail = (_dev(A2, "A2"), _dev(W2, "W2", A2.dtype), _dev(bias2, "bias2", A2.dtype) if bias2 is not None else None, M2, N2, K2,
            rows_per_batch2, heads2, dh2, len(kinds2), k2, d2, n_pad2, scale0_2, dtype_code(A2.dtype), _stream())
    if fold is None:
        head = (None, None, 0, 0, 0, 0, 0, 0, 0, None, None, 0, 0.0, None, None, None, None, None, 0.0)
        flops, tag = fl2, f"None {M2}x{N2}x{K2}"
    else:
        A, W = fold["A"], fold["W"]
        M, K = A.shape
        N = W.shape[0]
        kinds, dsts = fold["kinds"], fold["dsts"]
        k = (C.c_int * len(kinds))(*kinds)
        d = (C.c_void_p * len(kinds))(*[_dev(t, "dst", A.dtype) for t in dsts])
        fa = _fold_args(fold["part"], fold["u"], fold["v"], fold["center"], fold["center_out"], M, N, K)
        head = (_dev(A, "A"), _dev(W, "W", A.dtype), M, N, K, fold["rows_per_batch"], fold["heads"], fold["dh"], len(kinds), k, d,
                fold["n_pad"], fold.get("scale0", 1.0), fa[0], fa[1], fa[2], fa[3], fa[4], fold["eps"])
        flops, tag = 2.0 * M * N * K + fl2, f"None {M}x{N}x{K}+{M2}x{N2}x{K2}"
    _timed(tag, flops, lambda: check(_lib.load().primx_linear_heads_fold_pair(*head, *tail), "primx_linear_heads_fold_pair"))


def linear_fold(A: torch.Tensor, W: torch.Tensor, out: torch.Tensor, part: torch.Tensor, u: torch.Tensor, v: torch.Tensor,
                center: torch.Tensor, center_out: torch.Tensor, eps: float, act: int = ACT_NONE,
                carry: Optional[torch.Tensor] = None) -> torch.Tensor:
    M, K = A.shape
    N = W.shape[0]
    if tuple(out.shape) != (M, N) or out.dtype != A.dtype:
        raise RuntimeError("linear_fold: out must be a 16-bit [M, N] tensor of A's dtype")
    fa = _fold_args(part, u, v, center, center_out, M, N, K)
    cp, cn = _range(carry)
    _timed(f"None {M}x{N}x{K}", 2.0 * M * N * K, lambda: check(_lib.load().primx_linear_fold(
        _dev(A, "A"), _dev(W, "W", A.dtype), _dev(out, "out"), M, N, K, act, fa[0], fa[1], fa[2], fa[3], fa[4], eps,
        dtype_code(A.dtype), cp, cn, _stream()), "primx_linear_fold"))
    return out


KEY_MASK_VALUE = -30000.0


def alloc_heads(B: int, H: int, n: int, dh: int, kind: int, dtype: torch.dtype, device, pad_to: int,
                role: Optional[str] = None) -> torch.Tensor:
    DP = padded_head_dim(dh)
    n_pad = round_up(n, pad_to)
    shape = {HEADS_ROWS: (B, H, n_pad, DP), HEADS_KROWS: (B, H, n_pad, DP + 8), HEADS_VT: (B, H, DP, n_pad)}[kind]
    exact = DP == dh and n_pad == n and kind != HEADS_KROWS
    buf = torch.empty(shape, dtype=dtype, device=device) if exact else torch.zeros(shape, dtype=dtype, device=device)
    if kind != HEADS_VT and DP > dh:
        if role == "q":
            buf[:, :, :, dh] = 1.0
        elif role == "k":
            if n_pad > n:
                buf[:, :, n:, dh] = KEY_MASK_VALUE
            if DP - dh >= 3:
                buf[:, :, :, dh + 1:dh + 3] = 1.0
    if kind == HEADS_VT and DP > dh:
        k = torch.arange(n, device=device)
        quad = (k >> 2) & 3
        pos = (k & ~15) | ((((quad & 1) << 1) | (quad >> 1)) << 2) | (k & 3)
        buf[:, :, dh, pos] = 1.0
    return buf


def bcast_keys(nkv: int) -> int:
    return 64 + (nkv % 64 if nkv > 64 else 0)


def attention(Qp: torch.Tensor, Kp: Optional[torch.Tensor], Vt: Optional[torch.Tensor], nq: int, nkv: int, dh: int, scale: float,
              out: Optional[torch.Tensor] = None, bcast: Optional[Tuple[torch.Tensor, torch.Tensor]] = None) -> torch.Tensor:
    B, H, nq_pad, DP = Qp.shape
    if bcast is not None:
        Kb, Vb = bcast
        b_from = 0 if Kp is None else Kp.shape[0]
        nkv_pad_b = Kb.shape[2]
        if Kb.shape != (1, H, nkv_pad_b, DP + 8) or Vb.shape != (1, H, DP, nkv_pad_b) or not 0 <= b_from < B:
            raise RuntimeError("attention: broadcast operand layout mismatch")
        if Kp is not None and (Vt is None or Vt.shape != (b_from, H, DP, Kp.shape[2]) or Kp.shape[1:] != (H, Kp.shape[2], DP + 8)):
            raise RuntimeError("attention: operand layout mismatch")
        nkv_pad = Kp.shape[2] if Kp is not None else nkv_pad_b
        if out is None:
            out = torch.empty(B, nq, H * dh, dtype=Qp.dtype, device=Qp.device)
        name = f"attn_kernel<{dtype_code(Qp.dtype)}, {padded_head_dim(dh) // 16}, {(dh + 31) // 32}, {int(padded_head_dim(dh) == dh)}, 0>"
        _timed(f"{name} {B * H}x{nq}x{nkv}x{dh}", 4.0 * B * H * nq * nkv * dh, lambda: check(_lib.load().primx_attention_bcast(
            _dev(Qp, "Qp"), _dev(Kp, "Kp", Qp.dtype) if Kp is not None else None, _dev(Vt, "Vt", Qp.dtype) if Kp is not None else None,
            _dev(out, "out", Qp.dtype), B, H, nq, nq_pad, nkv, nkv_pad, dh, scale, _dev(Kb, "Kb", Qp.dtype), _dev(Vb, "Vb", Qp.dtype),
            b_from, nkv_pad_b, dtype_code(Qp.dtype), _stream()), "primx_attention_bcast"))
        return out
    nkv_pad = Kp.shape[2]
    if Vt.shape != (B, H, DP, nkv_pad) or Kp.shape != (B, H, nkv_pad, DP + 8):
        raise RuntimeError("attention: operand layout mismatch")
    if out is None:
        out = torch.empty(B, nq, H * dh, dtype=Qp.dtype, device=Qp.device)
    small = dh == 32 and nq <= 64 and nkv <= 64 and nq_pad == 64 and nkv_pad == 64
    name = f"attn64_kernel<{dtype_code(Qp.dtype)}>" if small else \
        f"attn_kernel<{dtype_code(Qp.dtype)}, {padded_head_dim(dh) // 16}, {(dh + 31) // 32}, {int(padded_head_dim(dh) == dh)}, 0>"
    _timed(f"{name} {B * H}x{nq}x{nkv}x{dh}", 4.0 * B * H * nq * nkv * dh, lambda: check(_lib.load().primx_attention(
        _dev(Qp, "Qp"), _dev(Kp, "Kp", Qp.dtype), _dev(Vt, "Vt", Qp.dtype), _dev(out, "out", Qp.dtype), B, H, nq,
        nq_pad, nkv, nkv_pad, dh, scale, dtype_code(Qp.dtype), _stream()), "primx_attention"))
    return out


def pack_heads(src: torch.Tensor, kind: int, pad_to: int, role: Optional[str] = None) -> torch.Tensor:
    B, M, H, dh = src.shape
    if src.stride(3) != 1 or not src.is_cuda:
        raise RuntimeError("pack_heads: last dim must be contiguous on a HIP device")
    dst = alloc_heads(B, H, M, dh, kind, src.dtype, src.device, pad_to, role)
    m_pad = dst.shape[3] if kind == HEADS_VT else dst.shape[2]
    check(_lib.load().primx_pack_heads(src.data_ptr(), src.stride(0), src.stride(1), src.stride(2), dst.data_ptr(),
                                       kind, B, M, H, dh, m_pad, dtype_code(src.dtype), _stream()), "primx_pack_heads")
    return dst


def memory_efficient_attention(q: torch.Tensor, k: torch.Tensor, v: torch.Tensor, attn_bias=None,
                               scale: Optional[float] = None) -> torch.Tensor:
    if attn_bias is not None:
        raise NotImplementedError("attn_bias is not used on the 3DTopia-XL path")
    B, Mq, H, dh = q.shape
    Mk = k.shape[1]
    Qp = pack_heads(q, HEADS_ROWS, BQ, "q")
    Kp = pack_heads(k, HEADS_KROWS, BKV, "k")
    Vt = pack_heads(v, HEADS_VT, BKV)
    out = attention(Qp, Kp, Vt, Mq, Mk, dh, dh ** -0.5 if scale is None else scale)
    return out.view(B, Mq, H, dh)


def cfg_combine(model_out: torch.Tensor, cfg_scale: float) -> torch.Tensor:
    B2 = model_out.shape[0]
    out = torch.empty((B2 // 2,) + tuple(model_out.shape[1:]), dtype=model_out.dtype, device=model_out.device)
    check(_lib.load().primx_cfg_combine(_dev(model_out, "model_out"), out.data_ptr(), dtype_code(model_out.dtype),
                                        out.numel(), cfg_scale, _stream()), "primx_cfg_combine")
    return out


def diffusion_step(x: torch.Tensor, model_out: torch.Tensor, coef: torch.Tensor, step: int, *, mean_type: int,
                   var_type: int, ancestral: bool, clip_denoised: bool,
                   noise: Optional[torch.Tensor]) -> Tuple[torch.Tensor, torch.Tensor]:
    B, nt, Cc = x.shape
    model_out = model_out.contiguous()
    sample = torch.empty_like(x)
    x0 = torch.empty_like(x)
    check(_lib.load().primx_diffusion_step(
        _dev(x, "x", torch.float32), _dev(model_out, "model_out"), dtype_code(model_out.dtype), B * nt, Cc,
        model_out.shape[-1], _dev(coef, "coef", torch.float32), step, mean_type, var_type, int(ancestral),
        int(clip_denoised), _dev(noise, "noise", torch.float32) if noise is not None else None,
        sample.data_ptr(), x0.data_ptr(), _stream()), "primx_diffusion_step")
    return sample, x0


def groupnorm_silu(x: torch.Tensor, gamma: torch.Tensor, beta: torch.Tensor, groups: int, eps: float,
                   silu: bool) -> torch.Tensor:
    P, V, Cc = x.shape
    out = torch.empty_like(x)
    _timed(f"groupnorm_silu {Cc}ch @{V}vox x{P}", 0.0, lambda: check(_lib.load().primx_groupnorm_silu(
        _dev(x, "x"), _dev(gamma, "gamma", torch.float32), _dev(beta, "beta", torch.float32), out.data_ptr(), P, V, Cc,
        groups, eps, int(silu), dtype_code(x.dtype), _stream()), "primx_groupnorm_silu"))
    return out


class PackedConv3:
    __slots__ = ("kind", "S", "Cin", "Cout", "Wp", "has_sc")

    def __init__(self, kind: str, S: int, Cin: int, Cout: int, Wp: torch.Tensor):
        self.kind, self.S, self.Cin, self.Cout, self.Wp, self.has_sc = kind, S, Cin, Cout, Wp, False


def pack_conv3(Wk: torch.Tensor, Cin: int, Wsc: Optional[torch.Tensor] = None) -> Optional[PackedConv3]:
    if not Wk.is_cuda or os.environ.get("PRIMX_CONV_REG", "1") == "0":
        return None
    Cout = Wk.shape[0]
    if Cin == 32 and Wk.shape[1] >= 864 and (Cout == 32 or Cout <= 16):
        NI = 2 if Cout == 32 else 1
        Wp = torch.empty(27 * NI * 16 * 32, dtype=Wk.dtype, device=Wk.device)
        with torch.cuda.device(Wk.device):
            check(_lib.load().primx_conv3d_s8c32_pack(_dev(Wk, "Wk"), Wp.data_ptr(), Cout, Wk.shape[1], dtype_code(Wk.dtype), _stream()),
                  "primx_conv3d_s8c32_pack")
        return PackedConv3("s8c32", 8, Cin, Cout, Wp)
    if Cin != 256 or Wk.shape[1] != 27 * 256:
        return None
    if Cout % 256 != 0 and Cout != 32:
        return None
    Wp = torch.empty_like(Wk)
    with torch.cuda.device(Wk.device):
        if Cout == 32:
            if Wsc is not None:
                Wp = torch.empty(28 * 8192, dtype=Wk.dtype, device=Wk.device)
            check(_lib.load().primx_conv3d_s8_pack(_dev(Wk, "Wk"), _dev(Wsc, "Wsc", Wk.dtype) if Wsc is not None else None, Wp.data_ptr(),
                                                   dtype_code(Wk.dtype), _stream()), "primx_conv3d_s8_pack")
            pc = PackedConv3("s8", 8, Cin, Cout, Wp)
            pc.has_sc = Wsc is not None
            return pc
        check(_lib.load().primx_conv3d_s4_pack(_dev(Wk, "Wk"), Wp.data_ptr(), Cout, dtype_code(Wk.dtype), _stream()), "primx_conv3d_s4_pack")
        return PackedConv3("s4", 4, Cin, Cout, Wp)


def conv3d_s8_fused(x_raw: torch.Tensor, Wp: PackedConv3, bias: Optional[torch.Tensor], part: torch.Tensor, up_bias: torch.Tensor,
                    gamma: torch.Tensor, beta: torch.Tensor, eps: float, sc_bias: Optional[torch.Tensor]):
    P, V, Cin = x_raw.shape
    if not (Wp.kind == "s8" and Wp.has_sc and V == 512 and Cin == 256):
        raise ValueError("conv3d_s8_fused: needs the 8^3 256 -> 32 image with the shortcut block")
    out = torch.empty(P, V, 32, dtype=x_raw.dtype, device=x_raw.device)
    sc = torch.empty(P, V, 32, dtype=x_raw.dtype, device=x_raw.device)
    tag = f"conv3_s8c256n32_kernel<{dtype_code(x_raw.dtype)}, 1> gn+256->32+sc @8^3 x{P}"
    _timed(tag, 2.0 * P * V * 32 * 28 * 256, lambda: check(_lib.load().primx_conv3d_s8_fused(
        _dev(x_raw, "x_raw"), _dev(Wp.Wp, "Wp", x_raw.dtype), _dev(bias, "bias", x_raw.dtype) if bias is not None else None,
        _dev(part, "part", torch.float32), _dev(up_bias, "up_bias", x_raw.dtype), _dev(gamma, "gamma", torch.float32),
        _dev(beta, "beta", torch.float32), float(eps), _dev(sc_bias, "sc_bias", x_raw.dtype) if sc_bias is not None else None,
        out.data_ptr(), sc.data_ptr(), P, dtype_code(x_raw.dtype), _stream()), "primx_conv3d_s8_fused"))
    return out, sc


def conv3_takes_groupnorm(Wp: Optional[PackedConv3], S: int, groups: int) -> bool:
    return Wp is not None and Wp.kind == "s8c32" and Wp.S == S and groups == Wp.Cin


def conv3d_k3(x: torch.Tensor, Wk: torch.Tensor, bias: Optional[torch.Tensor], S: int,
              res: Optional[torch.Tensor] = None, res_scale: float = 1.0, Wp: Optional[PackedConv3] = None,
              gn: Optional[Tuple[torch.Tensor, torch.Tensor, float]] = None) -> torch.Tensor:
    P, V, Cin = x.shape
    Cout, Kpad = Wk.shape
    out = torch.empty(P, V, Cout, dtype=x.dtype, device=x.device)
    bias_p = _dev(bias, "bias", x.dtype) if bias is not None else None
    res_p = _dev(res, "res", x.dtype) if res is not None else None
    tag, flops = f"conv3d_k3 {Cin}->{Cout} @{S}^3 x{P}", 2.0 * P * V * Cout * 27 * Cin
    if gn is not None and not conv3_takes_groupnorm(Wp, S, Cin):
        raise ValueError("conv3d_k3: gn= needs the 8^3 / 32-channel kernel (pack_conv3) and one channel per group")
    if Wp is not None and Wp.S == S and Wp.Cin == Cin and Wp.Cout == Cout and Wp.kind == "s8c32":
        tag = f"conv3_s8c32_kernel<{dtype_code(x.dtype)}, {2 if Cout == 32 else 1}> {'gn+' if gn else ''}{Cin}->{Cout} @{S}^3 x{P}"
        g_p = _dev(gn[0], "gamma", torch.float32) if gn else None
        b_p = _dev(gn[1], "beta", torch.float32) if gn else None
        _timed(tag, flops, lambda: check(_lib.load().primx_conv3d_s8c32_packed(
            _dev(x, "x"), _dev(Wp.Wp, "Wp", x.dtype), bias_p, g_p, b_p, float(gn[2]) if gn else 0.0, res_p, res_scale, out.data_ptr(),
            P, Cout, dtype_code(x.dtype), _stream()), "primx_conv3d_s8c32_packed"))
        return out
    if Wp is not None and Wp.S == S and Wp.Cin == Cin and Wp.Cout == Cout:
        if Wp.kind == "s4":
            tag = f"conv3_s4c256_kernel<{dtype_code(x.dtype)}, 0> {Cin}->{Cout} @{S}^3 x{P}"
            _timed(tag, flops, lambda: check(_lib.load().primx_conv3d_s4_packed(
                _dev(x, "x"), _dev(Wp.Wp, "Wp", x.dtype), bias_p, res_p, res_scale, out.data_ptr(), P, Cout, dtype_code(x.dtype),
                _stream()), "primx_conv3d_s4_packed"))
        else:
            tag = f"conv3_s8c256n32_kernel<{dtype_code(x.dtype)}, 0> {Cin}->{Cout} @{S}^3 x{P}"
            _timed(tag, flops, lambda: check(_lib.load().primx_conv3d_s8_packed(
                _dev(x, "x"), _dev(Wp.Wp, "Wp", x.dtype), bias_p, res_p, res_scale, out.data_ptr(), P, dtype_code(x.dtype),
                _stream()), "primx_conv3d_s8_packed"))
        return out
    _timed(tag, flops, lambda: check(_lib.load().primx_conv3d_k3(
        _dev(x, "x"), _dev(Wk, "Wk", x.dtype), bias_p, res_p, res_scale, out.data_ptr(), P, S, Cin, Cout, Kpad,
        dtype_code(x.dtype), _stream()), "primx_conv3d_k3"))
    return out


def linear_residual(A: torch.Tensor, W: torch.Tensor, bias: Optional[torch.Tensor],
                    res: Optional[torch.Tensor], scale: float) -> torch.Tensor:
    M, K = A.shape
    N = W.shape[0]
    out = torch.empty(M, N, dtype=A.dtype, device=A.device)
    _timed(f"linear_residual {M}x{N}x{K}", 2.0 * M * N * K, lambda: check(_lib.load().primx_linear_residual(
        _dev(A, "A"), _dev(W, "W", A.dtype), _dev(bias, "bias", A.dtype) if bias is not None else None,
        _dev(res, "res", A.dtype) if res is not None else None, scale, out.data_ptr(), M, N, K, dtype_code(A.dtype),
        _stream()), "primx_linear_residual"))
    return out


def conv_in(z: torch.Tensor, pq_scale: float, pq_bias: float, W: torch.Tensor, bias: torch.Tensor, S: int,
            dtype: torch.dtype) -> torch.Tensor:
    P = z.shape[0]
    Cout = W.shape[0]
    out = torch.empty(P, S * S * S, Cout, dtype=dtype, device=z.device)
    check(_lib.load().primx_conv_in(_dev(z, "z", torch.float32), pq_scale, pq_bias, _dev(W, "W", torch.float32),
                                    _dev(bias, "bias", torch.float32), out.data_ptr(), P, S, Cout,
                                    dtype_code(dtype), _stream()), "primx_conv_in")
    return out


def pack_convt_s4(Wt: torch.Tensor) -> Optional[torch.Tensor]:
    if tuple(Wt.shape) != (8 * 256, 256) or not Wt.is_cuda or os.environ.get("PRIMX_CONV_REG", "1") == "0":
        return None
    Wp = torch.empty_like(Wt)
    with torch.cuda.device(Wt.device):
        check(_lib.load().primx_convtranspose_s4_pack(_dev(Wt, "Wt"), Wp.data_ptr(), dtype_code(Wt.dtype), _stream()),
              "primx_convtranspose_s4_pack")
    return Wp


def convtranspose_k2s2(x: torch.Tensor, Wt: torch.Tensor, bias: torch.Tensor, S: int, Wp: Optional[torch.Tensor] = None,
                       want_stats: bool = False):
    P, V, Cin = x.shape
    Cout = Wt.shape[0] // 8
    out = torch.empty(P, 8 * V, Cout, dtype=x.dtype, device=x.device)
    if Wp is not None and S == 4 and Cin == 256 and Cout == 256:
        part = torch.empty(P, 16, 32, 2, dtype=torch.float32, device=x.device) if want_stats else None
        _timed(f"convt_s4c256_kernel<{dtype_code(x.dtype)}> {Cin}->{Cout} @{S}^3 x{P}", 2.0 * P * V * 8 * Cout * Cin, lambda: check(
            _lib.load().primx_convtranspose_s4_packed(_dev(x, "x"), _dev(Wp, "Wp", x.dtype), _dev(bias, "bias", x.dtype), out.data_ptr(),
                                                      part.data_ptr() if part is not None else None, P, dtype_code(x.dtype),
                                                      _stream()), "primx_convtranspose_s4_packed"))
        return (out, part) if want_stats else out
    if want_stats:
        raise ValueError("convtranspose_k2s2: statistics come only from the packed 4^3 kernel (pack_convt_s4)")
    _timed(f"convtranspose_k2s2 {Cin}->{Cout} @{S}^3 x{P}", 2.0 * P * V * 8 * Cout * Cin, lambda: check(
        _lib.load().primx_convtranspose_k2s2(_dev(x, "x"), _dev(Wt, "Wt", x.dtype), _dev(bias, "bias", x.dtype),
                                             out.data_ptr(), P, S, Cin, Cout, dtype_code(x.dtype), _stream()),
        "primx_convtranspose_k2s2"))
    return out


def group_stats(part: torch.Tensor, bias: torch.Tensor, eps: float, count: int = 4096) -> torch.Tensor:
    acc = torch.zeros_like(part[:, 0])
    for i in range(part.shape[1]):
        acc = acc + part[:, i]
    shift = bias.float()[0::8].view(1, 32)
    m = acc[..., 0] / count
    var = (acc[..., 1] / count - m * m).clamp_min(0.0)
    return torch.stack([shift + m, torch.rsqrt(var + eps)], dim=-1)


def vae_output(x: torch.Tensor, denorm: bool, sdf_div: float = 5.0) -> torch.Tensor:
    P, V, Cc = x.shape
    out = torch.empty(P, Cc, V, dtype=torch.float32, device=x.device)
    check(_lib.load().primx_vae_output(_dev(x, "x"), out.data_ptr(), P, V, Cc, int(denorm), sdf_div,
                                       dtype_code(x.dtype), _stream()), "primx_vae_output")
    return out


def latent_denorm(x: torch.Tensor, mean: torch.Tensor, std: torch.Tensor, nf: float, n_srt: int = 4):
    C = x.shape[-1]
    rows = x.numel() // C
    srt = torch.empty(*x.shape[:-1], n_srt, dtype=torch.float32, device=x.device)
    z = torch.empty(*x.shape[:-1], C - n_srt, dtype=torch.float32, device=x.device)
    check(_lib.load().primx_latent_denorm(_dev(x, "x", torch.float32), _dev(mean, "mean", torch.float32),
                                          _dev(std, "std", torch.float32), float(nf), srt.data_ptr(), z.data_ptr(),
                                          rows, C, n_srt, _stream()), "primx_latent_denorm")
    return srt, z


def vit_tokens(patches: torch.Tensor, cls: torch.Tensor, pos: torch.Tensor, reg: Optional[torch.Tensor]) -> torch.Tensor:
    B, npatch, D = patches.shape
    R = 0 if reg is None else reg.shape[0]
    out = torch.empty(B, 1 + R + npatch, D, dtype=torch.float32, device=patches.device)
    check(_lib.load().primx_vit_tokens(_dev(patches, "patches", torch.float32), _dev(cls, "cls", torch.float32),
                                       _dev(pos, "pos", torch.float32),
                                       _dev(reg, "reg", torch.float32) if reg is not None else None, out.data_ptr(), B,
                                       npatch, R, D, _stream()), "primx_vit_tokens")
    return out


def gemm_f32(A: torch.Tensor, W: torch.Tensor, bias: Optional[torch.Tensor], out: Optional[torch.Tensor] = None,
             act: int = ACT_NONE, out_scale: float = 1.0, gate: Optional[torch.Tensor] = None,
             rows_per_batch: int = 0) -> torch.Tensor:
    M, K = A.shape
    N = W.shape[0]
    if W.shape[1] != K:
        raise RuntimeError("gemm_f32: operand mismatch")
    if gate is not None:
        if out is None or gate.stride(-1) != 1 or gate.dtype != torch.float32 or not gate.is_cuda:
            raise RuntimeError("gemm_f32: the gated form updates `out` in place and needs a last-dim-contiguous fp32 gate")
    elif out is None:
        out = torch.empty(M, N, dtype=torch.float32, device=A.device)
    _timed("gemm_f32_kernel", 2.0 * M * N * K, lambda: check(_lib.load().primx_gemm_f32(
        _dev(A, "A", torch.float32), _dev(W, "W", torch.float32),
        _dev(bias, "bias", torch.float32) if bias is not None else None, _dev(out, "out", torch.float32), M, N, K, act,
        out_scale, gate.data_ptr() if gate is not None else None, gate.stride(0) if gate is not None else 0,
        rows_per_batch, _stream()), "primx_gemm_f32"))
    return out


def attention_f32(q: torch.Tensor, k: torch.Tensor, v: torch.Tensor, scale: Optional[float] = None) -> torch.Tensor:
    B, Mq, H, dh = q.shape
    Mk = k.shape[1]
    if k.shape != (B, Mk, H, dh) or v.shape != (B, Mk, H, dh):
        raise RuntimeError("attention_f32: q / k / v must be [B, M, H, dh] with equal B, H, dh")
    for t, name in ((q, "q"), (k, "k"), (v, "v")):
        if t.dtype != torch.float32 or not t.is_cuda or t.stride(3) != 1:
            raise RuntimeError(f"attention_f32: {name} must be an fp32 HIP tensor with a contiguous last dim")
    out = torch.empty(B, Mq, H, dh, dtype=torch.float32, device=q.device)
    strides = [(C.c_int64 * 3)(t.stride(0), t.stride(1), t.stride(2)) for t in (q, k, v)]
    _dev(out, "out", torch.float32)
    _timed("attn_f32_kernel", 4.0 * B * H * Mq * Mk * dh, lambda: check(_lib.load().primx_attention_f32(
        q.data_ptr(), k.data_ptr(), v.data_ptr(), out.data_ptr(), B, H, Mq, Mk, dh, strides[0], strides[1], strides[2],
        dh ** -0.5 if scale is None else scale, _stream()), "primx_attention_f32"))
    return out


def layernorm_modulate_f32(x: torch.Tensor, shift: torch.Tensor, scale: torch.Tensor, rows_per_batch: int,
                           eps: float = 1e-6, out: Optional[torch.Tensor] = None) -> torch.Tensor:
    rows, D = x.shape
    if shift.stride(-1) != 1 or scale.stride(-1) != 1 or shift.stride(0) != scale.stride(0) \
            or shift.dtype != torch.float32 or scale.dtype != torch.float32:
        raise RuntimeError("layernorm_modulate_f32: shift/scale must be fp32, last-dim contiguous, equal row strides")
    if out is None:
        out = torch.empty_like(x)
    check(_lib.load().primx_layernorm_modulate_f32(_dev(x, "x", torch.float32), shift.data_ptr(), scale.data_ptr(),
                                                   shift.stride(0), _dev(out, "out", torch.float32), rows, rows_per_batch,
                                                   D, eps, _stream()), "primx_layernorm_modulate_f32")
    return out


def silu_f32(x: torch.Tensor) -> torch.Tensor:
    out = torch.empty_like(x)
    check(_lib.load().primx_silu_f32(_dev(x, "x", torch.float32), out.data_ptr(), x.numel(), _stream()), "primx_silu_f32")
    return out
```

include/primx_hip.h:

```cpp
#ifndef PRIMX_HIP_H
#define PRIMX_HIP_H

#include <stdint.h>

#ifdef __cplusplus
extern "C" {
#endif

#define PRIMX_ABI_VERSION 30

#define PRIMX_F32 0
#define PRIMX_F16 1
#define PRIMX_BF16 2

#define PRIMX_OK 0
#define PRIMX_EINVAL (-1)
#define PRIMX_ELAUNCH (-2)

#define PRIMX_ACT_NONE 0
#define PRIMX_ACT_GELU_TANH 1
#define PRIMX_ACT_GELU_ERF 2

#define PRIMX_HEADS_ROWS 0
#define PRIMX_HEADS_VT 1
#define PRIMX_HEADS_KROWS 2

int primx_abi_version(void);
const char* primx_last_error(void);
const char* primx_last_gemm_kernel(void);

int primx_padded_head_dim(int dh);


int primx_layernorm_modulate(const float* x, const void* shift, const void* scale, int64_t mod_stride,
                             void* out, int dtype, int rows, int rows_per_batch, int D, float eps,
                             const void* pf0, int64_t pf0_bytes, const void* pf1, int64_t pf1_bytes, void* stream);

int primx_timestep_embedding(const int64_t* t, const float* freqs, float* emb, int B, int dim, void* stream);

int primx_vit_tokens(const float* patches, const float* cls, const float* pos, const float* reg, float* out, int B, int np,
                     int R, int D, void* stream);

int primx_point_features(const float* x, int64_t row_stride, const float* freqs, float* feat, int64_t feat_stride, int T,
                         int F, void* stream);

int primx_prefetch(const void* ptr, int64_t bytes, void* stream);
int primx_silu_cast(const float* in, void* out, int dtype, int64_t n, void* stream);

int primx_cast16(const float* in, void* out, int dtype, int64_t n, void* stream);

int primx_linear_f32(const float* in, const float* W, const float* bias, float* out, float* out2, int M, int N, int K,
                     int act_out, void* stream);


int primx_linear(const void* A, const void* W, const void* bias, void* out, int M, int N, int K, int dtype,
                 int act, float out_scale, const void* prefetch, int64_t prefetch_bytes, void* stream);

int primx_linear_gate_residual(const void* A, const void* W, const void* bias, const void* gate,
                               int64_t gate_stride, float* x, int M, int N, int K, int rows_per_batch,
                               int dtype, const void* prefetch, int64_t prefetch_bytes, void* stream);

int primx_linear_gate_residual_ln(const void* A, const void* W, const void* bias, const void* gate, int64_t gate_stride,
                                  float* x, int M, int N, int K, int rows_per_batch, const void* ln_shift, const void* ln_scale,
                                  int64_t ln_mod_stride, void* ln_out, float ln_eps, void* sync, int64_t sync_words, int dtype,
                                  const void* prefetch, int64_t prefetch_bytes, void* stream);
int primx_ln_sync_timeouts(void);


int primx_linear_f32out(const void* A, const void* W, const void* bias, float* out, int M, int N, int K, int bias_from_row,
                        int dtype, void* stream);

typedef struct PrimxF32outProblem {
    const void* A;
    const void* W;
    const void* bias;
    float* out;
    int N;
    int first_wg;
} PrimxF32outProblem;
int primx_linear_f32out_group(const PrimxF32outProblem* probs, int n_probs, int total_wg, int M, int K, int bias_from_row, int dtype,
                              void* stream);

int primx_row_stats(const float* x, int rows, int D, float eps, float* stats, void* stream);

int primx_linear_gate_residual_fold(const void* A, const void* W, const void* bias, const void* gate, int64_t gate_stride,
                                    float* x, int M, int N, int K, int rows_per_batch, const void* next_scale,
                                    int64_t next_mod_stride, const float* center, void* a16_out, float* part_out, int dtype,
                                    const void* prefetch, int64_t prefetch_bytes, void* stream);

int primx_linear_heads_fold(const void* A, const void* W, int M, int N, int K, int rows_per_batch, int heads, int dh, int n_seg,
                            const int* kind, void* const* dst, int n_pad, float scale0, const float* part, const float* u,
                            const float* v, const float* center, float* center_out, float eps, int dtype, const void* prefetch,
                            int64_t prefetch_bytes, void* stream);

int primx_linear_heads_fold_pair(const void* A, const void* W, int M, int N, int K, int rows_per_batch, int heads, int dh, int n_seg,
                                 const int* kind, void* const* dst, int n_pad, float scale0, const float* part, const float* u,
                                 const float* v, const float* center, float* center_out, float eps,
                                 const void* A2, const void* W2, const void* bias2, int M2, int N2, int K2, int rows_per_batch2,
                                 int heads2, int dh2, int n_seg2, const int* kind2, void* const* dst2, int n_pad2, float scale0_2,
                                 int dtype, void* stream);

int primx_linear_fold(const void* A, const void* W, void* out, int M, int N, int K, int act, const float* part, const float* u,
                      const float* v, const float* center, float* center_out, float eps, int dtype, const void* prefetch,
                      int64_t prefetch_bytes, void* stream);

int primx_linear_heads(const void* A, const void* W, const void* bias, int M, int N, int K, int rows_per_batch,
                       int heads, int dh, int n_seg, const int* kind, void* const* dst, int n_rep,
                       int rep_batches, int n_pad, float scale0, int dtype, const void* prefetch, int64_t prefetch_bytes,
                       void* stream);


int primx_attention(const void* Qp, const void* Kp, const void* Vt, void* out, int B, int H, int nq, int nq_pad,
                    int nkv, int nkv_pad, int dh, float scale, int dtype, void* stream);
int primx_attention_bcast(const void* Qp, const void* Kp, const void* Vt, void* out, int B, int H, int nq, int nq_pad, int nkv,
                          int nkv_pad, int dh, float scale, const void* Kb, const void* Vb, int b_from, int nkv_pad_b, int dtype,
                          void* stream);


typedef struct PrimxDitBlockFold {
    const void *w_q, *b_q, *w_cproj, *b_cproj, *w_qkv, *w_proj, *b_proj, *w_fc1, *w_fc2, *b_fc2;
    const void *Kc, *Vc, *Kb, *Vb;
    const float *uv_q, *uv_qkv, *uv_fc1;
    const void *carry_q, *carry_cproj, *carry_fc1, *carry_fc2;
    int64_t carry_q_bytes, carry_cproj_bytes, carry_fc1_bytes, carry_fc2_bytes;
} PrimxDitBlockFold;

typedef struct PrimxDitForwardFold {
    int dtype, Be, N, D, H, dh, hidden, depth, L, nq_pad, nkv_pad_c, nkv_pad_b, b_from, step, n_steps;
    float ln_eps, scale;
    float* h;
    void *xn, *att, *hid, *Qc, *Qs, *Ks, *Vs;
    const void* mod;
    float *center0, *center1, *part;
    const void *kv_A, *kv_W, *kv_bias;
    int kv_rows, kv_rows_per_batch, kv_K;
} PrimxDitForwardFold;

int primx_dit_blocks_fold(const PrimxDitForwardFold* f, const PrimxDitBlockFold* blocks, void* stream);

int primx_pack_heads(const void* src, int64_t sb, int64_t sm, int64_t sh, void* dst, int kind, int B, int M,
                     int H, int dh, int m_pad, int dtype, void* stream);


int primx_cfg_combine(const void* in, void* out, int dtype, int64_t n, float s, void* stream);

int primx_diffusion_step(const float* x, const void* model_out, int out_dtype, int64_t n_rows, int C, int c_out,
                         const float* coef, int step, int mean_type, int var_type, int ancestral, int clip,
                         const float* noise, float* sample, float* pred_xstart, void* stream);


int primx_groupnorm_silu(const void* in, const float* gamma, const float* beta, void* out, int P, int V, int C,
                         int groups, float eps, int silu, int dtype, void* stream);

int primx_conv3d_k3(const void* in, const void* Wk, const void* bias, const void* res, float res_scale,
                    void* out, int P, int S, int Cin, int Cout, int Kpad, int dtype, void* stream);

int primx_conv3d_s4_pack(const void* Wk, void* Wp, int Cout, int dtype, void* stream);
int primx_conv3d_s4_packed(const void* in, const void* Wp, const void* bias, const void* res, float res_scale, void* out,
                           int P, int Cout, int dtype, void* stream);

int primx_conv3d_s8_pack(const void* Wk, const void* Wsc, void* Wp, int dtype, void* stream);
int primx_conv3d_s8_packed(const void* in, const void* Wp, const void* bias, const void* res, float res_scale, void* out,
                           int P, int dtype, void* stream);
int primx_conv3d_s8_fused(const void* in_raw, const void* Wp28, const void* bias, const float* part, const void* up_bias,
                          const float* gamma, const float* beta, float eps, const void* sc_bias, void* out, void* sc_out, int P,
                          int dtype, void* stream);

int primx_conv3d_s8c32_pack(const void* Wk, void* Wp, int Cout, int Kpad, int dtype, void* stream);
int primx_conv3d_s8c32_packed(const void* in, const void* Wp, const void* bias, const float* gamma, const float* beta, float eps,
                              const void* res, float res_scale, void* out, int P, int Cout, int dtype, void* stream);

int primx_convtranspose_s4_pack(const void* Wt, void* Wp, int dtype, void* stream);
int primx_convtranspose_s4_packed(const void* in, const void* Wp, const void* bias, void* out, float* part, int P, int dtype,
                                  void* stream);

int primx_linear_residual(const void* A, const void* W, const void* bias, const void* res, float scale, void* out,
                          int M, int N, int K, int dtype, void* stream);

int primx_conv_in(const float* in, float pq_scale, float pq_bias, const float* W, const float* bias, void* out,
                  int P, int S, int Cout, int dtype, void* stream);

int primx_convtranspose_k2s2(const void* in, const void* Wt, const void* bias, void* out, int P, int S, int Cin,
                             int Cout, int dtype, void* stream);

int primx_vae_output(const void* in, float* out, int P, int V, int C, int denorm, float sdf_div, int dtype,
                     void* stream);

int primx_latent_denorm(const float* x, const float* mean, const float* stdv, float nf, float* srt, float* z,
                        int64_t rows, int C, int n_srt, void* stream);


int primx_primsdf_query(const float* pts, const float* srt, const float* feat, const float* lin, float* out, int n, int P,
                        int S, int C, int eval_fill, void* stream);


int primx_mcubes_workspace(int nx, int ny, int nz, int64_t* bytes);
int primx_mcubes_count(const float* vol, int nx, int ny, int nz, float iso, void* ws, int64_t ws_bytes, int64_t* totals,
                       void* stream);
int primx_mcubes_emit(const float* vol, int nx, int ny, int nz, float iso, const void* ws, int64_t ws_bytes, int64_t nverts,
                      int64_t ntris, float* verts, float* normals, int* tris, void* stream);

int primx_noise_filter(const float* srt, int P, uint8_t* keep, void* stream);


int primx_texbake_labels(const float* v, const float* n, const int* f, int V, int F, int* label, void* stream);

int primx_texbake_components_workspace(int F, int U, int64_t* bytes);
int primx_texbake_components(const int* node, int F, int U, void* ws, int64_t ws_bytes, int* comp, int64_t* n_comp,
                             void* stream);

int primx_texbake_raster_workspace(int W, int H, int64_t* bytes);
int primx_texbake_raster(const int* uv, const int* ft, int NUV, int F, int W, int H, int* face_id, int* cover, void* ws,
                         int64_t ws_bytes, int64_t* totals, void* stream);

int primx_texbake_compact(const int* face_id, int W, int H, const void* ws, int64_t ws_bytes, const int* uv, const int* ft,
                          int NUV, const float* v, const int* f, int V, int F, int64_t n, int* texel, float* points,
                          void* stream);

int primx_texbake_fill_workspace(int W, int H, int64_t* bytes);
int primx_texbake_fill(const float* attr, const int* texel, int64_t n, const int* face_id, int W, int H, int radius,
                       int band, void* ws, int64_t ws_bytes, uint8_t* albedo, uint8_t* metallic_roughness, void* stream);


int primx_meshclean_workspace(int V, int F, int64_t* bytes);
int primx_meshclean_merge(const float* v, const int* f, int V, int F, double v_pct, void* ws, int64_t ws_bytes, int* centre,
                          int64_t* rounds, float* radius, void* stream);
int primx_meshclean_faces(const float* v, const int* fr, const int* tid, int V, int F, void* ws, int64_t ws_bytes, int* out_f,
                          int64_t* n_out, void* stream);
int primx_meshclean_components(const float* v, const int* f, const int* node, const int* comp, int V, int F, int U,
                               int n_comp, int min_f, double min_d, int repair, void* ws, int64_t ws_bytes, int* out_f,
                               int* out_node, int64_t* cand_key, int64_t* counts, void* stream);
int primx_meshclean_edges(const int* f, const int* node, int F, int U, const int64_t* cand_key, int64_t n_cand, void* ws,
                          int64_t ws_bytes, int* out_f, int64_t* n_out, void* stream);
int primx_meshclean_fans(const int* f, const int* fan, int V, int F, int n_fans, void* ws, int64_t ws_bytes, int* out_f,
                         int64_t* vmap, int64_t* counts, void* stream);


int primx_meshdecim_workspace(int V, int F, int64_t* bytes);
int primx_meshdecim_edges(const int* f, const int* node, const int* sv, int V, int F, int U, int* ecnt, int* vcls,
                          int* first, int* last, void* stream);
int primx_meshdecim_quadrics(const float* v, const int* f, const int* node, const int* order, const int* first,
                             const int* last, const int* ecnt, int V, int F, int U, double* p, double* Q, void* stream);
int primx_meshdecim_costs(const double* p, const double* Q, const int64_t* ukeys, const int* ecnt, const int* vcls, int V,
                          int U, int optimalplacement, double* x, double* cost, int64_t* key, int* valid, void* stream);
int primx_meshdecim_select(const double* p, const int* f, const int* node, const int* order, const int* first,
                           const int* last, const int64_t* ukeys, const int* ecnt, const int* valid, const double* x,
                           const int64_t* cand, int V, int F, int U, int K, int64_t* m1, int* ok, int* sel, void* stream);
int primx_meshdecim_collapse(double* p, double* Q, int* f, const int* order, const int* first, const int* last,
                             const int64_t* ukeys, const int* ecnt, const double* x, const int64_t* cand, const int* sel,
                             int V, int F, int U, int K, int target, void* ws, int64_t ws_bytes, int* out_f,
                             int64_t* counts, void* stream);
int primx_meshdecim_finish(const double* p, const int* f, int V, int F, void* ws, int64_t ws_bytes, float* out_v, int* out_f,
                           int64_t* vmap, int64_t* n_out, void* stream);
int primx_meshdecim_normals(const float* v, const int* f, const int* sv, const int* order, int V, int F, void* ws,
                            int64_t ws_bytes, float* normals, void* stream);


int primx_compute_raydirs(const float* viewpos, const float* viewrot, const float* focal, const float* princpt,
                          const float* pixelcoords, float volradius, float* raypos, float* raydir, float* tminmax, int N,
                          int H, int W, void* stream);

int primx_raymarch(const float* raypos, const float* raydir, const float* tminmax, float stepsize, const float* primpos,
                   const float* primrot, const float* primscale, const float* tplate, float* rayrgba, int N, int H, int W,
                   int K, int TD, int TH, int TW, float fadescale, float fadeexp, void* stream);


int primx_gemm_f32(const float* A, const float* W, const float* bias, float* out, int M, int N, int K, int act,
                   float out_scale, const float* gate, int64_t gate_stride, int rows_per_batch, void* stream);

int primx_attention_f32(const float* q, const float* k, const float* v, float* out, int B, int H, int Nq, int Nkv,
                        int dh, const int64_t* q_strides, const int64_t* k_strides, const int64_t* v_strides, float scale,
                        void* stream);

int primx_layernorm_modulate_f32(const float* x, const float* shift, const float* scale, int64_t mod_stride, float* out,
                                 int rows, int rows_per_batch, int D, float eps, void* stream);

int primx_silu_f32(const float* in, float* out, int64_t n, void* stream);

#ifdef __cplusplus
}
#endif
#endif
```

Baseline: 121.3.

## Fuse DiT step head and tail into single kernels with CFG combine

Adds a step_head kernel that does the input projection (K=68 to D=1152), writes h for both CFG halves, and computes the first block's layernorm-modulate and row stats in one launch. Adds a step_tail kernel that fuses the final layernorm-modulate, the output linear and the CFG combine. Both skip the matching launches in the block driver. This cuts kernel launches and intermediate HBM round-trips per denoise step, at the cost of shape-specialised kernels (D=1152 only) and new ABI plumbing.

```diff
diff --git a/3dtopia-xl_amd/_lib.py b/3dtopia-xl_amd/_lib.py
--- a/3dtopia-xl_amd/_lib.py
+++ b/3dtopia-xl_amd/_lib.py
@@ -10,7 +10,7 @@
 F32, F16, BF16 = 0, 1, 2
 ACT_NONE, ACT_GELU_TANH, ACT_GELU_ERF = 0, 1, 2
 HEADS_ROWS, HEADS_VT, HEADS_KROWS = 0, 1, 2
-ABI_VERSION = 30
+ABI_VERSION = 31
 
 _p, _i, _l, _f, _d = C.c_void_p, C.c_int, C.c_int64, C.c_float, C.c_double
 
@@ -32,7 +32,8 @@
                                   "b_from", "step", "n_steps")] + \
                [("ln_eps", _f), ("scale", _f)] + \
                [(n, _p) for n in ("h", "xn", "att", "hid", "Qc", "Qs", "Ks", "Vs", "mod", "center0", "center1", "part")] + \
-               [(n, _p) for n in ("kv_A", "kv_W", "kv_bias")] + [(n, _i) for n in ("kv_rows", "kv_rows_per_batch", "kv_K")]
+               [(n, _p) for n in ("kv_A", "kv_W", "kv_bias")] + [(n, _i) for n in ("kv_rows", "kv_rows_per_batch", "kv_K")] + \
+               [(n, _i) for n in ("head_done", "tail_fused")]
 
 
 SIGNATURES = {
@@ -58,6 +59,10 @@
     "primx_ln_sync_timeouts": [],
     "primx_linear_f32out": [_p, _p, _p, _p, _i, _i, _i, _i, _i, _p],
     "primx_row_stats": [_p, _i, _i, _f, _p, _p],
+    "primx_step_head_supported": [_i, _i],
+    "primx_step_head": [_p, _p, _p, _p, _p, _p, _l, _p, _p, _i, _i, _i, _i, _i, _f, _i, _p],
+    "primx_step_tail_supported": [_i, _i],
+    "primx_step_tail": [_p, _p, _p, _l, _p, _p, _p, _i, _i, _i, _i, _f, _f, _i, _p],
     "primx_linear_gate_residual_fold": [_p, _p, _p, _p, _l, _p, _i, _i, _i, _i, _p, _l, _p, _p, _p, _i, _p, _l, _p],
     "primx_linear_heads_fold": [_p, _p, _i, _i, _i, _i, _i, _i, _i, C.POINTER(_i), C.POINTER(_p), _i, _f, _p, _p, _p, _p, _p, _f,
                                 _i, _p, _l, _p],
@@ -130,11 +135,13 @@
 _MESHDECIM_ENTRY_POINTS: set = {"primx_meshdecim_workspace", "primx_meshdecim_edges", "primx_meshdecim_quadrics",
                                 "primx_meshdecim_costs", "primx_meshdecim_select", "primx_meshdecim_collapse",
                                 "primx_meshdecim_finish", "primx_meshdecim_normals"}
-_AB_ABI_VERSIONS: tuple = (21, 22, 23, 24, 25, 26, 27, 28, 29)
+_STEP_ENTRY_POINTS: set = {"primx_step_head_supported", "primx_step_head", "primx_step_tail_supported", "primx_step_tail"}
+_AB_ABI_VERSIONS: tuple = (21, 22, 23, 24, 25, 26, 27, 28, 29, 30)
 _fold_available: dict = {}
 _blocks_call: dict = {}
 _kv_ride: dict = {}
 _f32out_group: dict = {}
+_step_fused: dict = {}
 
 _lib: Optional[C.CDLL] = None
 
@@ -188,6 +195,8 @@
             continue
         if got < 30 and name in _MESHDECIM_ENTRY_POINTS:
             continue
+        if got < 31 and name in _STEP_ENTRY_POINTS:
+            continue
         fn = getattr(lib, name)
         fn.argtypes = argtypes
         fn.restype = _RESTYPES.get(name, C.c_int)
@@ -195,6 +204,7 @@
     _blocks_call[path] = got >= 24
     _kv_ride[path] = got >= 25
     _f32out_group[path] = got >= 26
+    _step_fused[path] = got >= 31
     if path == LIB_PATH:
         _lib = lib
     return lib
@@ -218,6 +228,11 @@
 def f32out_group_available() -> bool:
     load()
     return _f32out_group.get(LIB_PATH, False)
+
+
+def step_fused_available() -> bool:
+    load()
+    return _step_fused.get(LIB_PATH, False)
 
 
 def check(status: int, name: str) -> None:
diff --git a/3dtopia-xl_amd/csrc/build.py b/3dtopia-xl_amd/csrc/build.py
--- a/3dtopia-xl_amd/csrc/build.py
+++ b/3dtopia-xl_amd/csrc/build.py
@@ -8,7 +8,7 @@
 from concurrent.futures import ThreadPoolExecutor
 
 HERE = os.path.dirname(os.path.abspath(__file__))
-SOURCES = ["rowops.hip", "gemm.hip", "attention.hip", "vae.hip", "primsdf.hip", "raymarch.hip", "fp32.hip", "conv3.hip", "conv3s8.hip", "conv3s8c32.hip", "convt.hip", "dit_host.hip", "mcubes.hip", "texbake.hip", "meshclean.hip", "meshdecim.hip"]
+SOURCES = ["rowops.hip", "step.hip", "gemm.hip", "attention.hip", "vae.hip", "primsdf.hip", "raymarch.hip", "fp32.hip", "conv3.hip", "conv3s8.hip", "conv3s8c32.hip", "convt.hip", "dit_host.hip", "mcubes.hip", "texbake.hip", "meshclean.hip", "meshdecim.hip"]
 HEADERS = ["common.h", "ln_row.h", "gemm288q_body.inc", "mc_tables.h", "block_scan.h", os.path.join("..", "..", "include", "primx_hip.h")]
 LIB = os.path.join(HERE, "libprimx_hip.so")
 MANIFEST = os.path.join(HERE, "build_manifest.json")
diff --git a/3dtopia-xl_amd/csrc/dit_host.hip b/3dtopia-xl_amd/csrc/dit_host.hip
--- a/3dtopia-xl_amd/csrc/dit_host.hip
+++ b/3dtopia-xl_amd/csrc/dit_host.hip
@@ -59,8 +59,10 @@
             PRIMX_FAIL("primx_dit_blocks_fold: block %d: null weight or table", i);
         const float *u, *v;
         if (i == 0) {
-            PRIMX_DIT_CALL(primx_layernorm_modulate(f->h, ch(0, 0), ch(0, 1), 0, f->xn, dt, T, N, D, f->ln_eps, nullptr, 0, nullptr, 0, stream));
-            PRIMX_DIT_CALL(primx_row_stats(f->h, T, D, f->ln_eps, center[0], stream));
+            if (!f->head_done) {
+                PRIMX_DIT_CALL(primx_layernorm_modulate(f->h, ch(0, 0), ch(0, 1), 0, f->xn, dt, T, N, D, f->ln_eps, nullptr, 0, nullptr, 0, stream));
+                PRIMX_DIT_CALL(primx_row_stats(f->h, T, D, f->ln_eps, center[0], stream));
+            }
             side = 0;
         }
         if (b.uv_q) {
@@ -103,6 +105,8 @@
         if (i + 1 < f->depth) {
             PRIMX_DIT_CALL(primx_linear_gate_residual_fold(f->hid, b.w_fc2, b.b_fc2, ch(i, 8), 0, f->h, T, D, f->hidden, N, ch(i + 1, 1), 0,
                                                            center[side], f->xn, f->part, dt, b.carry_fc2, b.carry_fc2_bytes, stream));
+        } else if (f->tail_fused) {
+            PRIMX_DIT_CALL(primx_linear_gate_residual(f->hid, b.w_fc2, b.b_fc2, ch(i, 8), 0, f->h, T, D, f->hidden, N, dt, nullptr, 0, stream));
         } else {
             PRIMX_DIT_CALL(primx_linear_gate_residual_ln(f->hid, b.w_fc2, b.b_fc2, ch(i, 8), 0, f->h, T, D, f->hidden, N, ch(f->depth, 0),
                                                          ch(f->depth, 1), 0, f->xn, f->ln_eps, nullptr, 0, dt, nullptr, 0, stream));
diff --git a/3dtopia-xl_amd/csrc/ln_row.h b/3dtopia-xl_amd/csrc/ln_row.h
--- a/3dtopia-xl_amd/csrc/ln_row.h
+++ b/3dtopia-xl_amd/csrc/ln_row.h
@@ -48,3 +48,43 @@
         *reinterpret_cast<V4*>(orow + c * 128) = o;
     }
 }
+
+template <int NCH4>
+__device__ __forceinline__ void ln_row32_stats(const f32x4 (&v)[NCH4], float eps, float& mean, float& rstd) {
+    constexpr int D = NCH4 * 128;
+    float s = 0.f;
+#pragma unroll
+    for (int c = 0; c < NCH4; ++c) s += (v[c][0] + v[c][1]) + (v[c][2] + v[c][3]);
+    mean = half_wave_sum(s) * (1.0f / D);
+    float q = 0.f;
+#pragma unroll
+    for (int c = 0; c < NCH4; ++c)
+#pragma unroll
+        for (int j = 0; j < 4; ++j) {
+            const float a = v[c][j] - mean;
+            q += a * a;
+        }
+    rstd = 1.0f / sqrtf(half_wave_sum(q) * (1.0f / D) + eps);
+}
+
+template <int DT, int NCH4>
+__device__ __forceinline__ void ln_row32_store(const f32x4 (&v)[NCH4], float mean, float rstd, const typename T16<DT>::S* __restrict__ sh,
+                                               const typename T16<DT>::S* __restrict__ sc, typename T16<DT>::S* __restrict__ orow, int l32) {
+    using S = typename T16<DT>::S;
+    using V4 = typename T16<DT>::V4;
+    sh += l32 * 4;
+    sc += l32 * 4;
+    orow += l32 * 4;
+#pragma unroll
+    for (int c = 0; c < NCH4; ++c) {
+        const V4 s4 = *reinterpret_cast<const V4*>(sc + c * 128);
+        const V4 h4 = *reinterpret_cast<const V4*>(sh + c * 128);
+        V4 o;
+#pragma unroll
+        for (int j = 0; j < 4; ++j) {
+            const float m1 = rnd16<DT>(1.0f + (float)s4[j]);
+            o[j] = (S)((v[c][j] - mean) * rstd * m1 + (float)h4[j]);
+        }
+        *reinterpret_cast<V4*>(orow + c * 128) = o;
+    }
+}
diff --git a/3dtopia-xl_amd/csrc/step.hip b/3dtopia-xl_amd/csrc/step.hip
--- /dev/null
+++ b/3dtopia-xl_amd/csrc/step.hip
@@ -0,0 +1,233 @@
+#include "common.h"
+#include "ln_row.h"
+
+template <int DT, int NCH4, int K>
+__global__ __launch_bounds__(256) void step_head_kernel(const float* __restrict__ x, const float* __restrict__ W, const float* __restrict__ bias,
+                                                        float* __restrict__ h, const typename T16<DT>::S* __restrict__ shift,
+                                                        const typename T16<DT>::S* __restrict__ scale, int64_t mod_stride,
+                                                        typename T16<DT>::S* __restrict__ xn, f32x2* __restrict__ stats, int rows,
+                                                        int rows_per_batch, int halves, float eps) {
+    typedef __attribute__((address_space(1))) const void GV;
+    typedef __attribute__((address_space(3))) void LV;
+    constexpr int D = NCH4 * 128;
+    constexpr int CH = 128 * K;
+    constexpr int NP = (NCH4 + 1) / 2;
+    constexpr int INST = CH * 4 / 1024;
+    static_assert(K % 4 == 0 && (K / 4) % 2 == 1, "weight rows: 16-byte pieces, an odd number of them (conflict-free ds_read_b128)");
+    static_assert((CH * 4) % 1024 == 0, "a chunk is whole LDS-DMA wave-instructions");
+    static_assert(8 * D <= 2 * CH, "the row tile is parked in stage 0");
+    __shared__ __attribute__((aligned(16))) float smem[4 * CH + K * 8];
+    float* const Xs = smem + 4 * CH;
+
+    const int tid = threadIdx.x, lane = tid & 63;
+    const int wave = __builtin_amdgcn_readfirstlane(tid >> 6);
+    const int g = wave >> 1, t = tid & 127;
+    const int m0 = (int)blockIdx.x * 8;
+
+    auto issue = [&](int p, int n_inst) {
+        const float* src = W + (int64_t)p * 2 * CH;
+        const int per_wave = (n_inst + 3) / 4;
+        for (int i = 0; i < per_wave; ++i) {
+            const int it = min(wave + 4 * i, n_inst - 1);
+            __builtin_amdgcn_global_load_lds((GV*)(uintptr_t)(src + it * 256 + lane * 4), (LV*)(smem + (p & 1) * 2 * CH + it * 256), 16, 0, 0);
+        }
+    };
+    auto pair_inst = [](int p) { return (2 * p + 1 < NCH4 ? 2 : 1) * INST; };
+
+    issue(0, pair_inst(0));
+    if (tid < 8 * (K / 4)) {
+        const int r = tid / (K / 4), k4 = tid - r * (K / 4);
+        const f32x4 v = *reinterpret_cast<const f32x4*>(x + (int64_t)min(m0 + r, rows - 1) * K + 4 * k4);
+#pragma unroll
+        for (int j = 0; j < 4; ++j) Xs[(4 * k4 + j) * 8 + r] = v[j];
+    }
+
+    float acc[NCH4][4];
+#pragma unroll
+    for (int c = 0; c < NCH4; ++c)
+#pragma unroll
+        for (int r = 0; r < 4; ++r) acc[c][r] = 0.f;
+
+#pragma unroll
+    for (int p = 0; p < NP; ++p) {
+        const bool two = 2 * p + 1 < NCH4;
+        const int c1 = two ? 2 * p + 1 : 2 * p;
+        if (p + 1 < NP) {
+            issue(p + 1, pair_inst(p + 1));
+            if (2 * (p + 1) + 1 < NCH4) asm volatile("s_waitcnt vmcnt(%0) lgkmcnt(0)\n\ts_barrier" ::"n"((2 * INST + 3) / 4) : "memory");
+            else asm volatile("s_waitcnt vmcnt(%0) lgkmcnt(0)\n\ts_barrier" ::"n"((INST + 3) / 4) : "memory");
+        } else {
+            asm volatile("s_waitcnt vmcnt(0) lgkmcnt(0)\n\ts_barrier" ::: "memory");
+        }
+        const float* w0 = smem + (p & 1) * 2 * CH + t * K;
+        const float* w1 = w0 + CH;
+#pragma unroll 2
+        for (int k4 = 0; k4 < K / 4; ++k4) {
+            const f32x4 wa = *reinterpret_cast<const f32x4*>(w0 + 4 * k4);
+            f32x4 wb = {0.f, 0.f, 0.f, 0.f};
+            if (two) wb = *reinterpret_cast<const f32x4*>(w1 + 4 * k4);
+#pragma unroll
+            for (int j = 0; j < 4; ++j) {
+                const f32x4 xv = *reinterpret_cast<const f32x4*>(&Xs[(4 * k4 + j) * 8 + 4 * g]);
+#pragma unroll
+                for (int r = 0; r < 4; ++r) {
+                    acc[2 * p][r] = fmaf(xv[r], wa[j], acc[2 * p][r]);
+                    if (two) acc[c1][r] = fmaf(xv[r], wb[j], acc[c1][r]);
+                }
+            }
+        }
+        asm volatile("s_waitcnt lgkmcnt(0)\n\ts_barrier" ::: "memory");
+    }
+
+    float* Hs = smem;
+    float bv[NCH4];
+#pragma unroll
+    for (int c = 0; c < NCH4; ++c) bv[c] = bias[128 * c + t];
+#pragma unroll
+    for (int c = 0; c < NCH4; ++c)
+#pragma unroll
+        for (int r = 0; r < 4; ++r) Hs[(4 * g + r) * D + 128 * c + t] = acc[c][r] + bv[c];
+    __syncthreads();
+
+    const int hw = tid >> 5, l32 = tid & 31;
+    const int row = m0 + hw;
+    if (row >= rows) return;
+    f32x4 v[NCH4];
+#pragma unroll
+    for (int c = 0; c < NCH4; ++c) v[c] = *reinterpret_cast<const f32x4*>(Hs + hw * D + 4 * l32 + 128 * c);
+    float mean, rstd;
+    ln_row32_stats<NCH4>(v, eps, mean, rstd);
+    const int b = row / rows_per_batch, nb = rows / rows_per_batch;
+    for (int hf = 0; hf < halves; ++hf) {
+        const int64_t orow = (int64_t)hf * rows + row;
+        float* hr = h + orow * D + 4 * l32;
+#pragma unroll
+        for (int c = 0; c < NCH4; ++c) *reinterpret_cast<f32x4*>(hr + 128 * c) = v[c];
+        if (stats && l32 == 0) stats[orow] = f32x2{mean, rstd};
+        const int64_t mrow = ((int64_t)hf * nb + b) * mod_stride;
+        ln_row32_store<DT, NCH4>(v, mean, rstd, shift + mrow, scale + mrow, xn + orow * D, l32);
+    }
+}
+
+extern "C" int primx_step_head_supported(int D, int K) { return D == 1152 && K == 68; }
+
+extern "C" int primx_step_head(const float* x, const float* W, const float* bias, float* h, const void* shift, const void* scale,
+                               int64_t mod_stride, void* xn, float* stats, int rows, int rows_per_batch, int D, int K, int halves, float eps,
+                               int dtype, void* stream) {
+    const char* name = "primx_step_head";
+    PRIMX_REQUIRE(x && W && bias && h && shift && scale && xn, "%s: null pointer", name);
+    PRIMX_REQUIRE(rows > 0 && rows_per_batch > 0 && rows % rows_per_batch == 0 && (halves == 1 || halves == 2),
+                  "%s: need rows > 0 in whole batch entries of rows_per_batch > 0 rows and 1 or 2 halves (rows %d, rows per batch entry %d, halves %d)",
+                  name, rows, rows_per_batch, halves);
+    PRIMX_REQUIRE(primx_step_head_supported(D, K), "%s: no kernel for D = %d, K = %d (primx_step_head_supported)", name, D, K);
+    PRIMX_REQUIRE(((uintptr_t)x | (uintptr_t)W | (uintptr_t)h) % 16 == 0, "%s: x, W and h must be 16-byte aligned", name);
+    PRIMX_REQUIRE((((uintptr_t)shift | (uintptr_t)scale | (uintptr_t)xn) & 7) == 0 && mod_stride % 4 == 0 && ((uintptr_t)stats & 7) == 0,
+                  "%s: shift, scale, xn and stats must be 8-byte aligned, the modulation row stride a multiple of 4", name);
+    PRIMX_DISPATCH_16(dtype, name, {
+        using S = typename T16<DT>::S;
+        hipLaunchKernelGGL((step_head_kernel<DT, 9, 68>), dim3((rows + 7) / 8), dim3(256), 0, (hipStream_t)stream, x, W, bias, h, (const S*)shift,
+                           (const S*)scale, mod_stride, (S*)xn, reinterpret_cast<f32x2*>(stats), rows, rows_per_batch, halves, eps);
+    });
+    PRIMX_CHECK_LAUNCH(name);
+    return PRIMX_OK;
+}
+
+template <int DT>
+__global__ __launch_bounds__(320) void step_tail_kernel(const float* __restrict__ h, const typename T16<DT>::S* __restrict__ shift,
+                                                        const typename T16<DT>::S* __restrict__ scale, int64_t mod_stride,
+                                                        const typename T16<DT>::S* __restrict__ W, const typename T16<DT>::S* __restrict__ bias,
+                                                        typename T16<DT>::S* __restrict__ out, int rows, int rows_per_batch, int N, float cfg,
+                                                        float eps) {
+    using S = typename T16<DT>::S;
+    using V8 = typename T16<DT>::V8;
+    typedef __attribute__((address_space(1))) const void GV;
+    typedef __attribute__((address_space(3))) void LV;
+    constexpr int NCH4 = 9, D = NCH4 * 128, RS = D + 8;
+    constexpr int WROWS = 160, STAGE = WROWS * 64, NST = 3, NK = D / 64;
+    __shared__ __attribute__((aligned(16))) S smem[32 * RS + NST * STAGE];
+    S* const As = smem;
+    S* const Wst = smem + 32 * RS;
+
+    const int tid = threadIdx.x, lane = tid & 63;
+    const int wave = __builtin_amdgcn_readfirstlane(tid >> 6);
+    const int lr = lane & 31, lg = lane >> 5;
+    const int m0 = (int)blockIdx.x * 16;
+
+    const S* gp[4];
+#pragma unroll
+    for (int i = 0; i < 4; ++i) {
+        const int row = 8 * (wave + 5 * i) + (lane >> 3);
+        const int c = (lane & 7) ^ ((row >> 1) & 7);
+        gp[i] = W + (int64_t)min(row, N - 1) * D + c * 8;
+    }
+    auto issue = [&](int kt, int stage) {
+#pragma unroll
+        for (int i = 0; i < 4; ++i)
+            __builtin_amdgcn_global_load_lds((GV*)(uintptr_t)(gp[i] + kt * 64), (LV*)(Wst + stage * STAGE + (wave + 5 * i) * 512), 16, 0, 0);
+    };
+#pragma unroll
+    for (int s0 = 0; s0 < NST; ++s0) issue(s0, s0);
+
+    const int nb = rows / rows_per_batch;
+    for (int i = tid >> 5; i < 32; i += 10) {
+        const int half = i >> 4, tok = min(m0 + (i & 15), rows - 1);
+        const int64_t mrow = ((int64_t)half * nb + tok / rows_per_batch) * mod_stride;
+        ln_row32<DT, NCH4>(h + ((int64_t)half * rows + tok) * D, shift + mrow, scale + mrow, As + i * RS, tid & 31, eps);
+    }
+    asm volatile("s_waitcnt vmcnt(0) lgkmcnt(0)\n\ts_barrier" ::: "memory");
+
+    f32x16 acc;
+#pragma unroll
+    for (int r = 0; r < 16; ++r) acc[r] = 0.f;
+    const S* arow = As + lr * RS + lg * 8;
+    const int wrow = 32 * wave + lr;
+    for (int kt = 0; kt < NK; ++kt) {
+        const int stage = kt % NST;
+        const S* Ws = Wst + stage * STAGE;
+#pragma unroll
+        for (int s = 0; s < 4; ++s) {
+            const V8 a = *reinterpret_cast<const V8*>(arow + kt * 64 + s * 16);
+            const V8 b = *reinterpret_cast<const V8*>(Ws + wrow * 64 + (((2 * s + lg) ^ ((wrow >> 1) & 7)) << 3));
+            acc = T16<DT>::mfma32(a, b, acc);
+        }
+        if (kt + 1 < NK) {
+            asm volatile("s_waitcnt vmcnt(4) lgkmcnt(0)\n\ts_barrier" ::: "memory");
+            issue(min(kt + NST, NK - 1), stage);
+        }
+    }
+    asm volatile("s_waitcnt vmcnt(0)" ::: "memory");
+
+    const int n = 32 * wave + lr;
+    if (n >= N) return;
+    const float bv = bias ? (float)bias[n] : 0.f;
+#pragma unroll
+    for (int r = 0; r < 8; ++r) {
+        const int m = m0 + (r & 3) + 8 * (r >> 2) + 4 * lg;
+        if (m >= rows) continue;
+        const float yc = rnd16<DT>(acc[r] + bv), yu = rnd16<DT>(acc[r + 8] + bv);
+        const float d = rnd16<DT>(yc - yu);
+        const float mm = rnd16<DT>(cfg * d);
+        out[(int64_t)m * N + n] = (S)(yu + mm);
+    }
+}
+
+extern "C" int primx_step_tail_supported(int D, int N) { return D == 1152 && N > 0 && N <= 160; }
+
+extern "C" int primx_step_tail(const float* h, const void* shift, const void* scale, int64_t mod_stride, const void* W, const void* bias,
+                               void* out, int rows, int rows_per_batch, int D, int N, float cfg_scale, float eps, int dtype, void* stream) {
+    const char* name = "primx_step_tail";
+    PRIMX_REQUIRE(h && shift && scale && W && out, "%s: null pointer", name);
+    PRIMX_REQUIRE(rows > 0 && rows_per_batch > 0 && rows % rows_per_batch == 0,
+                  "%s: need rows > 0 in whole batch entries of rows_per_batch > 0 rows (rows %d, rows per batch entry %d)", name, rows, rows_per_batch);
+    PRIMX_REQUIRE(primx_step_tail_supported(D, N), "%s: no kernel for D = %d, N = %d (primx_step_tail_supported)", name, D, N);
+    PRIMX_REQUIRE(((uintptr_t)h | (uintptr_t)W) % 16 == 0, "%s: h and W must be 16-byte aligned", name);
+    PRIMX_REQUIRE((((uintptr_t)shift | (uintptr_t)scale) & 7) == 0 && mod_stride % 4 == 0,
+                  "%s: shift and scale must be 8-byte aligned, the modulation row stride a multiple of 4", name);
+    PRIMX_DISPATCH_16(dtype, name, {
+        using S = typename T16<DT>::S;
+        hipLaunchKernelGGL((step_tail_kernel<DT>), dim3((rows + 15) / 16), dim3(320), 0, (hipStream_t)stream, h, (const S*)shift, (const S*)scale,
+                           mod_stride, (const S*)W, (const S*)bias, (S*)out, rows, rows_per_batch, N, cfg_scale, eps);
+    });
+    PRIMX_CHECK_LAUNCH(name);
+    return PRIMX_OK;
+}
diff --git a/3dtopia-xl_amd/dit.py b/3dtopia-xl_amd/dit.py
--- a/3dtopia-xl_amd/dit.py
+++ b/3dtopia-xl_amd/dit.py
@@ -125,6 +125,8 @@
         self.fold_max_steps = int(os.environ.get("PRIMX_DIT_FOLD_MAX_STEPS", "128"))
         self.blocks_call = os.environ.get("PRIMX_DIT_BLOCKS_CALL", "1") != "0"
         self.kv_ride = os.environ.get("PRIMX_DIT_KV_RIDE", "1") != "0"
+        self.step_head = os.environ.get("PRIMX_DIT_STEP_HEAD", "1") != "0"
+        self.step_tail = os.environ.get("PRIMX_DIT_STEP_TAIL", "1") != "0"
         self._fold_fp16_used = False
         self.block_probe: Optional[list] = None
         self._side: Dict = {}
@@ -493,7 +495,7 @@
         A[:, :, 1] = v[:, :, :, 0].permute(1, 2, 0, 3)
         return A
 
-    def _forward16(self, x, t, y, dt, null_half: bool):
+    def _forward16(self, x, t, y, dt, null_half: bool, cfg_scale: Optional[float] = None):
         B, N, Cin = x.shape
         Be = 2 * B if null_half else B
         L, Dc = y.shape[1], y.shape[2]
@@ -506,7 +508,6 @@
 
         xf = x.reshape(B * N, Cin).float().contiguous()
         h = torch.empty(T, D, dtype=torch.float32, device=dev)
-        self._embed_tokens(xf, h[:B * N], h[B * N:] if null_half else None)
         plan = self._t_plan
         if plan is not None and plan["row"] is not None:
             mod = self._modulation_table(plan, dt, pk)[plan["row"]:plan["row"] + 1].expand(Be, -1)
@@ -551,7 +552,8 @@
             if dedup:
                 ops.linear_heads(cs["null16"], pk["w_kv_all"], pk["b_kv_all"], Ln, H, dh, [HEADS_KROWS, HEADS_VT], [Kn, Vn],
                                  Kn.shape[2], n_rep=self.depth, rep_batches=1)
-            cs["kv_valid"], cs["kv_id"] = True, (Kc.data_ptr(), Vc.data_ptr())
+            if cond_rows:
+                cs["kv_valid"], cs["kv_id"] = True, (Kc.data_ptr(), Vc.data_ptr())
         Qs = self._heads("Qs", Be, N, HEADS_ROWS, dt, dev, ops.BQ)
         Ks = self._heads("Ks", Be, N, HEADS_KROWS, dt, dev, ops.BQ)
         Vs = self._heads("Vs", Be, N, HEADS_VT, dt, dev, ops.BQ)
@@ -585,6 +587,19 @@
                 self._fold_ws = {wk: ops.fold_workspace(T, D, dev)}
             fcent, fpart = self._fold_ws[wk]
 
+        w_emb, b_emb = self.x_embedder.weight.detach(), self.x_embedder.bias
+        head_done = (bool(self.step_head) and self.depth > 0 and type(self)._embed_tokens is DiT._embed_tokens and wpf != 1
+                     and ops.PROFILE is None and b_emb is not None and B * N > 8 and ops.step_head_ok(D, Cin)
+                     and mod.data_ptr() % 8 == 0 and mod.stride(0) % 4 == 0 and w_emb.is_contiguous() and w_emb.dtype == torch.float32)
+        if head_done:
+            ops.step_head(xf, w_emb, b_emb.detach(), h, mod[:, :D], mod[:, D:2 * D], N, xn, self.LN_EPS,
+                          stats=fcent[0] if fold_uv is not None else None)
+        else:
+            self._embed_tokens(xf, h[:B * N], h[B * N:] if null_half else None)
+        tail_fused = (bool(self.step_tail) and null_half and cfg_scale is not None and ops.PROFILE is None and self.block_probe is None
+                      and ops.step_tail_ok(D, self.out_channels) and mod.data_ptr() % 8 == 0 and mod.stride(0) % 4 == 0
+                      and (base * mod.element_size()) % 8 == 0)
+
         fside: Dict[int, int] = {}
 
         def warm(*wts):
@@ -617,10 +632,13 @@
             def uv(s):
                 return uvs[s][0, prow], uvs[s][1, prow]
             if not fuse or i == 0:
-                ops.layernorm_modulate(hh, ch[0], ch[1], N, xh, self.LN_EPS, prefetch=warm(w["w_q"], w["w_cproj"]))
+                first_done = i == 0 and head_done
+                if not first_done:
+                    ops.layernorm_modulate(hh, ch[0], ch[1], N, xh, self.LN_EPS, prefetch=warm(w["w_q"], w["w_cproj"]))
                 if folded:
                     fside[b0] = 0
-                    ops.row_stats(hh, self.LN_EPS, fc_in())
+                    if not first_done:
+                        ops.row_stats(hh, self.LN_EPS, fc_in())
             bc = min(b1, B) if collapse else b1
             if bc > b0:
                 if folded and i > 0:
@@ -681,7 +699,7 @@
                                               carry=carry(blocks[i + 1]["w_q"]))
             else:
                 ops.linear_gate_residual(hid[r0:r1], w["w_fc2"], w["b_fc2"], ch[8], hh, N,
-                                         carry=None if last else carry(blocks[i + 1]["w_q"]), ln=ln_of(*nxt))
+                                         carry=None if last else carry(blocks[i + 1]["w_q"]), ln=None if last and tail_fused else ln_of(*nxt))
 
         two_streams = bool(self.cfg_streams and null_half and self.depth and ops.PROFILE is None)
         one_call = (not two_streams and fold_uv is not None and self.blocks_call and sync is None and ops.PROFILE is None
@@ -734,6 +752,7 @@
             if ride:
                 f.kv_A, f.kv_W, f.kv_bias = y16.data_ptr(), pk["w_kv_all"].data_ptr(), pk["b_kv_all"].data_ptr()
                 f.kv_rows, f.kv_rows_per_batch, f.kv_K = Bkv * Lk, Lk, Dc
+            f.head_done, f.tail_fused = int(head_done), int(tail_fused)
             ops._dev(h, "h", torch.float32)
             _lib.check(_lib.load().primx_dit_blocks_fold(C.byref(f), fd["desc"], ops._stream()), "primx_dit_blocks_fold")
         else:
@@ -747,10 +766,15 @@
                         "row_std_max": float(rs.max()), "row_mean_abs_max": float(h.mean(-1).abs().max()),
                         "next_operand_abs_max": float(xn.float().abs().max()), "next_operand_finite": bool(torch.isfinite(xn.float()).all())})
 
+        if need_kv and ride:
+            cs["kv_valid"], cs["kv_id"] = True, (Kc.data_ptr(), Vc.data_ptr())
+        if tail_fused:
+            out = ops.step_tail(h, fin_mod[0], fin_mod[1], N, pk["w_final"], pk["b_final"], float(cfg_scale), self.LN_EPS)
+            return out.view(B, N, self.out_channels)
         if not (fuse and self.depth):
             ops.layernorm_modulate(h, fin_mod[0], fin_mod[1], N, xn, self.LN_EPS)
-        out = ops.linear(xn, pk["w_final"], pk["b_final"])
-        return out.view(Be, N, self.out_channels)
+        out = ops.linear(xn, pk["w_final"], pk["b_final"]).view(Be, N, self.out_channels)
+        return out if cfg_scale is None else ops.cfg_combine(out, float(cfg_scale))
 
     def _forward_fp32(self, x, t, y):
         if self._packed_only:
@@ -806,7 +830,7 @@
     def forward_with_cfg(self, x, t, y, cfg_scale=0.0, precision_dtype=torch.float32, enable_amp=False):
         self._check_inputs(x)
         if enable_amp and precision_dtype in (torch.float16, torch.bfloat16):
-            model_out = self._forward16(x, t, y, precision_dtype, null_half=True)
+            return self._forward16(x, t, y, precision_dtype, null_half=True, cfg_scale=float(cfg_scale))
         else:
             y_null = self.null_cond_embedding.detach().to(y.dtype).expand_as(y)
             model_out = self.forward(torch.cat([x, x], dim=0), torch.cat([t, t], dim=0), torch.cat([y, y_null], dim=0),
diff --git a/3dtopia-xl_amd/ops.py b/3dtopia-xl_amd/ops.py
--- a/3dtopia-xl_amd/ops.py
+++ b/3dtopia-xl_amd/ops.py
@@ -292,6 +292,54 @@
         raise RuntimeError("row_stats: out must be [rows, 2] fp32")
     check(_lib.load().primx_row_stats(_dev(x, "x", torch.float32), rows, D, eps, _dev(out, "stats", torch.float32), _stream()),
           "primx_row_stats")
+    return out
+
+
+def step_head_ok(D: int, K: int) -> bool:
+    return _lib.step_fused_available() and bool(_lib.load().primx_step_head_supported(D, K))
+
+
+def step_tail_ok(D: int, N: int) -> bool:
+    return _lib.step_fused_available() and bool(_lib.load().primx_step_tail_supported(D, N))
+
+
+def _halves_modulation(shift: torch.Tensor, scale: torch.Tensor, out: torch.Tensor, entries: int, name: str) -> None:
+    _check_modulation(shift, scale, out)
+    if shift.shape[0] != entries or scale.shape[0] != entries or shift.data_ptr() % 8 or scale.data_ptr() % 8 or shift.stride(0) % 4:
+        raise RuntimeError(f"{name}: shift / scale must be [{entries}, D] views, 8-byte aligned, row stride a multiple of 4")
+
+
+def step_head(x: torch.Tensor, W: torch.Tensor, b: torch.Tensor, h: torch.Tensor, shift: torch.Tensor, scale: torch.Tensor,
+              rows_per_batch: int, xn: torch.Tensor, eps: float, stats: Optional[torch.Tensor] = None) -> None:
+    rows, K = x.shape
+    D = W.shape[0]
+    halves = h.shape[0] // max(rows, 1)
+    if h.shape != (halves * rows, D) or halves not in (1, 2) or tuple(xn.shape) != tuple(h.shape) or tuple(W.shape) != (D, K) or tuple(b.shape) != (D,):
+        raise RuntimeError("step_head: shape mismatch")
+    if rows % rows_per_batch or (stats is not None and tuple(stats.shape) != (halves * rows, 2)):
+        raise RuntimeError("step_head: rows must be whole batch entries and stats [halves * rows, 2]")
+    _halves_modulation(shift, scale, xn, halves * (rows // rows_per_batch), "step_head")
+    check(_lib.load().primx_step_head(
+        _dev(x, "x", torch.float32), _dev(W, "W", torch.float32), _dev(b, "b", torch.float32), _dev(h, "h", torch.float32),
+        shift.data_ptr(), scale.data_ptr(), shift.stride(0), _dev(xn, "xn"), _dev(stats, "stats", torch.float32) if stats is not None else None,
+        rows, rows_per_batch, D, K, halves, eps, dtype_code(xn.dtype), _stream()), "primx_step_head")
+
+
+def step_tail(h: torch.Tensor, shift: torch.Tensor, scale: torch.Tensor, rows_per_batch: int, W: torch.Tensor, bias: Optional[torch.Tensor],
+              cfg_scale: float, eps: float, out: Optional[torch.Tensor] = None) -> torch.Tensor:
+    rows2, D = h.shape
+    rows, N = rows2 // 2, W.shape[0]
+    if rows2 != 2 * rows or rows % rows_per_batch or tuple(W.shape) != (N, D) or (bias is not None and tuple(bias.shape) != (N,)):
+        raise RuntimeError("step_tail: shape mismatch")
+    if out is None:
+        out = torch.empty(rows, N, dtype=W.dtype, device=h.device)
+    elif tuple(out.shape) != (rows, N) or out.dtype != W.dtype:
+        raise RuntimeError("step_tail: out must be a 16-bit [rows, N] tensor of W's dtype")
+    _halves_modulation(shift, scale, out, 2 * (rows // rows_per_batch), "step_tail")
+    check(_lib.load().primx_step_tail(
+        _dev(h, "h", torch.float32), shift.data_ptr(), scale.data_ptr(), shift.stride(0), _dev(W, "W"),
+        _dev(bias, "bias", W.dtype) if bias is not None else None, _dev(out, "out"), rows, rows_per_batch, D, N, cfg_scale, eps,
+        dtype_code(W.dtype), _stream()), "primx_step_tail")
     return out
 
 
diff --git a/include/primx_hip.h b/include/primx_hip.h
--- a/include/primx_hip.h
+++ b/include/primx_hip.h
@@ -7,7 +7,7 @@
 extern "C" {
 #endif
 
-#define PRIMX_ABI_VERSION 30
+#define PRIMX_ABI_VERSION 31
 
 #define PRIMX_F32 0
 #define PRIMX_F16 1
@@ -83,6 +83,15 @@
 
 int primx_row_stats(const float* x, int rows, int D, float eps, float* stats, void* stream);
 
+int primx_step_head_supported(int D, int K);
+int primx_step_head(const float* x, const float* W, const float* bias, float* h, const void* shift, const void* scale,
+                    int64_t mod_stride, void* xn, float* stats, int rows, int rows_per_batch, int D, int K, int halves, float eps,
+                    int dtype, void* stream);
+
+int primx_step_tail_supported(int D, int N);
+int primx_step_tail(const float* h, const void* shift, const void* scale, int64_t mod_stride, const void* W, const void* bias,
+                    void* out, int rows, int rows_per_batch, int D, int N, float cfg_scale, float eps, int dtype, void* stream);
+
 int primx_linear_gate_residual_fold(const void* A, const void* W, const void* bias, const void* gate, int64_t gate_stride,
                                     float* x, int M, int N, int K, int rows_per_batch, const void* next_scale,
                                     int64_t next_mod_stride, const float* center, void* a16_out, float* part_out, int dtype,
@@ -134,6 +143,7 @@
     float *center0, *center1, *part;
     const void *kv_A, *kv_W, *kv_bias;
     int kv_rows, kv_rows_per_batch, kv_K;
+    int head_done, tail_fused;
 } PrimxDitForwardFold;
 
 int primx_dit_blocks_fold(const PrimxDitForwardFold* f, const PrimxDitBlockFold* blocks, void* stream);
```

Measured after the change: 121.1. Within noise of the previous version (-0.2%).
